# thilinarmtb/lsbench

Hardware: AMD Instinct MI355X
Metric: cg_solves_per_sec (higher is better)
Workload: dtype f64

## Files before the change

### include/lsbench_hip.h

```cpp
#ifndef LSBENCH_HIP_H
#define LSBENCH_HIP_H

#include "lsbench.h"
#include <stddef.h>

#ifdef __cplusplus
extern "C" {
#endif


struct lsbench {
  char *matrix;
  lsbench_solver_t solver;
  lsbench_ordering_t ordering;
  lsbench_precision_t precision;
  unsigned verbose, trials;
};

struct csr {
  unsigned nrows, base;
  unsigned *offs, *cols;
  double *vals;
};

// ... 49 lines not shown
  int overlap;
  int spmv_tune;
  int spmv_grid;
  int reorder;
  int krylov;
  int restart;
  int verbose;
  int ngpus;
  int verify;
  int cheb_degree;
  int block_size;
  int precision;
  int persistent;
  double comm_deadline_s;
  int fsai_power;
  int blas1_nt;
};
enum { LSB_PREC_FP64 = 0, LSB_PREC_MIXED = 1 };

struct lsb_hip_result {
  unsigned iters;
  int status;
  double relres;
  double seconds;
  double spmv_ms;
  unsigned spmv_samples;
  unsigned corrections;
  double true_relres;
  unsigned spmvs;
};

void lsb_hip_opts_default(struct lsb_hip_opts *o);
void lsb_hip_set_opts(const struct lsb_hip_opts *o);
void lsb_hip_get_opts(struct lsb_hip_opts *o);
void lsb_hip_last_result(struct lsb_hip_result *res);
int lsb_hip_device_count(void);


void lsb_csr_free(struct csr *A);
struct csr *lsb_csr_symmetrize_upper(const struct csr *A);
struct csr *lsb_csr_copy_base0(const struct csr *A);
struct csr *lsb_csr_row_slice(const struct csr *A, unsigned r0, unsigned r1);
int lsb_csr_partition_rows(const struct csr *A, unsigned nparts,
                           unsigned *bounds);
unsigned lsb_csr_row_blocks(const struct csr *A, unsigned cap,
                            unsigned **rowblk);
void lsb_csr_block_lanes(const struct csr *A, const unsigned *rowblk,
                         unsigned nblk, unsigned char *lanes);
struct csr *lsb_csr_pad_lines(const struct csr *S, unsigned slice, unsigned *nx, unsigned *nxp, int **map);
int lsb_csr_rcm(const struct csr *S, unsigned *perm);
struct csr *lsb_csr_permute_sym(const struct csr *S, const unsigned *perm);
unsigned lsb_csr_bandwidth(const struct csr *S);
struct lsb_panel_csr {
  unsigned npanels, width, npairs, nrows;
  unsigned *pair_begin;
  unsigned *pair_row;
  unsigned *offs;
  unsigned *cols;
  double *vals;
};
struct lsb_panel_csr *lsb_csr_panelize(const struct csr *A, unsigned width);
void lsb_panel_csr_free(struct lsb_panel_csr *P);
#define LSB_BIN_CHUNK 2048
struct lsb_binned {
  unsigned nbins, width, nrows, nchunks;
  unsigned chunk_cap;
  unsigned long long nnz;
  unsigned *bin_chunk;
  unsigned *chunk_begin;
  unsigned *rows;
  unsigned *cols;
  double *vals;
};
struct lsb_binned *lsb_csr_binize(const struct csr *A, unsigned width);
void lsb_binned_free(struct lsb_binned *B);
#define LSB_PB_COLS 8192
#define LSB_PB_ROWS 2048
struct lsb_pb {
  unsigned nrows, ncols_lo, nchunks, nbins, nitems, npieces;
  unsigned cols, rows;
  unsigned long long nnz;
  unsigned long long nent;
  double *vals;
  unsigned short *colw;
  unsigned *grp_first;
  unsigned long long *grp_mask;
  unsigned *delta;
  unsigned *item;
  unsigned *bin_ptr;
  unsigned short *roww;
};
struct lsb_pb *lsb_csr_pbize2(const struct csr *A, unsigned cols, unsigned rows);
struct lsb_pb *lsb_csr_pbize(const struct csr *A);
void lsb_pb_free(struct lsb_pb *P);
int lsb_pb_check(const struct lsb_pb *P, unsigned long long prod_len, unsigned long long roww_len, int deep,
                 char *why, size_t whylen);
struct lsb_fsai_pattern {
  unsigned n, cap;
  unsigned long long nnz;
  unsigned *offs, *cols;
};
#define LSB_FSAI_CAP 128
struct lsb_fsai_pattern *lsb_csr_fsai_pattern(const struct csr *S, int power, unsigned cap);
void lsb_fsai_pattern_free(struct lsb_fsai_pattern *P);
#define LSB_SELL_ROWS 128
struct lsb_sell {
  unsigned nrows, nslice;
  unsigned long long stored;
  unsigned *sptr;
  int *cols;
  double *vals;
  short *codes;
  int *sbase;
  unsigned ncode_slots;
};
unsigned long long lsb_csr_sell_stored(const struct csr *A);
struct lsb_sell *lsb_csr_sellize(const struct csr *A);
struct lsb_sell *lsb_csr_sellize16(const struct csr *A, unsigned row_begin);
void lsb_sell_free(struct lsb_sell *S);
struct lsb_sell_vc {
  unsigned long long nslots;
  unsigned nval_slots;
  int *slots;
  double *vconst;
  double *vals;
};
struct lsb_sell_vc *lsb_sell16_value_slots(const struct lsb_sell *S);
void lsb_sell_vc_free(struct lsb_sell_vc *V);
#define LSB_TMPL_SLOTS 8
struct lsb_sell_tmpl {
  int nslots;
  int shaped;
  int base[LSB_TMPL_SLOTS];
  int kidx[LSB_TMPL_SLOTS];
  int kind[LSB_TMPL_SLOTS];
  int pad_[2];
  double cst[LSB_TMPL_SLOTS];
};
struct lsb_sell_tmpls {
  unsigned nslice, ntmpl, nfar;
  unsigned long long covered, shaped;
  unsigned long long nmask;
  unsigned long long kept_read;
  unsigned char *tid;
  unsigned *vbase;
  unsigned long long *mask;
  struct lsb_sell_tmpl *t;
};
struct lsb_sell_tmpls *lsb_sell16_templates(const struct lsb_sell *S, const struct lsb_sell_vc *V);
void lsb_sell_tmpls_free(struct lsb_sell_tmpls *T);
int lsb_tmpl_check(const struct lsb_sell *S, const struct lsb_sell_vc *V, const struct lsb_sell_tmpls *T,
                   unsigned row_begin, unsigned nrows, unsigned xlen, int deep, char *why, size_t whylen);
#define LSB_TMPL_COL_MAX 16
#define LSB_TMPL_COL_LOCKSTEP 0x80000000u
struct lsb_tmpl_cols {
  unsigned nitem, kmax, period;
  unsigned s_lo, s_hi;
  unsigned xbeg[9];
  unsigned *item;
  unsigned long long in_cols;
  int centre0;
};
struct lsb_tmpl_cols *lsb_sell_tmpl_columns(const struct lsb_sell_tmpls *T, unsigned period, unsigned kmax);
struct lsb_tmpl_cols *lsb_sell_tmpl_columns_range(const struct lsb_sell_tmpls *T, unsigned period, unsigned kmax,
                                                  unsigned s_lo, unsigned s_hi);
void lsb_tmpl_cols_free(struct lsb_tmpl_cols *C);
int lsb_tmpl_cols_check(const struct lsb_sell_tmpls *T, const struct lsb_tmpl_cols *C, char *why, size_t whylen);
double lsb_csr_mean_scatter(const struct csr *A, unsigned row_begin);
void lsb_csr_col_hull(const struct csr *A, unsigned *lo, unsigned *hi);
struct lsb_xfer {
  int peer;
  size_t offset, count;
};
void lsb_plan_exchange(int me, int nall, const unsigned *hull,
                       struct lsb_xfer *recv, int *nrecv,
                       struct lsb_xfer *send, int *nsend);
struct csr *lsbench_matrix_synth(const char *spec, unsigned r0, unsigned r1,
                                 unsigned *n_global);


typedef struct lsb_hip_solver lsb_hip_solver;

lsb_hip_solver *lsb_hip_solver_create(const struct csr *A,
                                      const struct lsb_hip_opts *o);
lsb_hip_solver *lsb_hip_solver_create_dist(const struct csr *A_rows,
                                           unsigned row_begin,
                                           unsigned n_global,
                                           const struct lsb_hip_opts *o);
void lsb_hip_solver_destroy(lsb_hip_solver *s);

int lsb_hip_solver_solve(lsb_hip_solver *s, const double *b, double *x,
                         struct lsb_hip_result *res);
int lsb_hip_solver_solve_dev(lsb_hip_solver *s, const double *d_b, double *d_x,
                             struct lsb_hip_result *res);
int lsb_hip_solver_spmv_dev(lsb_hip_solver *s, const double *d_x, double *d_y);
int lsb_hip_solver_time_spmv(lsb_hip_solver *s, int warm, int reps,
                             double *ms_avg);
int lsb_hip_solver_jacobi_sweep_dev(lsb_hip_solver *s, double w,
                                    const double *d_b, double *d_x);

unsigned lsb_hip_solver_nrows_local(const lsb_hip_solver *s);
int lsb_hip_solver_padded(const lsb_hip_solver *s);
unsigned lsb_hip_solver_nrows_global(const lsb_hip_solver *s);
unsigned long long lsb_hip_solver_nnz_local(const lsb_hip_solver *s);
unsigned lsb_hip_solver_nblocks(const lsb_hip_solver *s);
int lsb_hip_solver_spmv_variant(const lsb_hip_solver *s);
unsigned lsb_hip_solver_spmv_flags(const lsb_hip_solver *s);
unsigned lsb_hip_solver_spmv_grid(const lsb_hip_solver *s);
unsigned lsb_hip_solver_spmv_period(const lsb_hip_solver *s);
unsigned long long lsb_hip_solver_spmv_col_slices(const lsb_hip_solver *s);
void lsb_hip_solver_sell_value_slots(const lsb_hip_solver *s, unsigned *kept, unsigned *total);
int lsb_hip_solver_overlaps(const lsb_hip_solver *s);
int lsb_hip_solver_comm(const lsb_hip_solver *s, double *p2p_us, double *rccl_us);
void lsb_hip_solver_comm_plan(const lsb_hip_solver *s, unsigned long long plan[8]);
int lsb_hip_solver_overlap(const lsb_hip_solver *s, double us[2]);
unsigned long long lsb_hip_solver_spmv_layout_bytes(const lsb_hip_solver *s);
unsigned long long lsb_hip_solver_iteration_bytes(const lsb_hip_solver *s);
int lsb_hip_solver_single_reduction(const lsb_hip_solver *s);
int lsb_hip_solver_fused_p(const lsb_hip_solver *s);
int lsb_hip_solver_blas1_nt(const lsb_hip_solver *s);
void *lsb_hip_stream(void);


#define LSB_HIP_UNIQUE_ID_BYTES 128
int lsb_hip_comm_get_unique_id(void *id128);
int lsb_hip_comm_init_rank(const void *id128, int nranks, int rank);
int lsb_hip_comm_destroy(void);
int lsb_hip_comm_rank(void);
int lsb_hip_comm_size(void);
int lsb_hip_comm_count(void);
int lsb_hip_comm_allreduce_sum_dev(double *d_buf, int count);
int lsb_hip_comm_barrier(void);


#define LSB_SPMV_FLAG_PREFETCH 1u
#define LSB_SPMV_FLAG_NT 2u
#define LSB_SPMV_FLAG_C16 4u
int lsb_hip_spmv_csr_f64(int variant, unsigned n, const int *d_offs,
                         const int *d_cols, const double *d_vals,
                         const int *d_rowblk, const unsigned char *d_blklanes,
                         unsigned nblk, unsigned mean_row_len, unsigned flags,
                         const double *d_x, double *d_y,
                         const double *d_xdot, double *d_dot, double *d_work,
                         void *stream);
unsigned lsb_hip_partials_capacity(void);
int lsb_hip_dot_f64(unsigned n, const double *d_a, const double *d_b,
                    double *d_out, double *d_work, void *stream);
int lsb_hip_nrm2_f64(unsigned n, const double *d_a, double *d_out,
                     double *d_work, void *stream);
int lsb_hip_axpy_f64(unsigned n, const double *d_alpha, const double *d_x,
                     double *d_y, void *stream);
int lsb_hip_xpay_f64(unsigned n, const double *d_beta, const double *d_x,
                     double *d_y, void *stream);
int lsb_hip_jacobi_setup_f64(unsigned n, unsigned row_begin, const int *d_offs,
                             const int *d_cols, const double *d_vals,
                             double *d_dinv, int *d_nzero, void *stream);
int lsb_hip_jacobi_apply_f64(unsigned n, const double *d_dinv,
                             const double *d_r, double *d_z, void *stream);

void *lsb_hip_malloc(size_t bytes);
void lsb_hip_free(void *d_ptr);
int lsb_hip_memcpy_h2d(void *d_dst, const void *src, size_t bytes);
int lsb_hip_memcpy_d2h(void *dst, const void *d_src, size_t bytes);
int lsb_hip_sync(void);

#ifdef __cplusplus
}
#endif

#endif
```

### lsbench_amd/_lib.py

```python
import ctypes as C
import os
import subprocess

_CSRC = os.path.join(os.path.dirname(os.path.abspath(__file__)), "csrc")
LIB_PATH = os.path.join(_CSRC, "liblsbench_hip.so")
CORE_PATH = os.path.join(_CSRC, "liblsbench_core.so")
CORE_SYMBOLS = ("lsbench_matrix_read", "lsbench_matrix_print", "lsbench_matrix_free", "lsbench_init",
                "lsbench_get_matrix_name", "lsbench_bench", "lsbench_finalize")

UNIQUE_ID_BYTES = 128

SOLVER_HIP = 6
OP_CHOLMOD_UPPER, OP_RAW = 0, 1
PRECOND_JACOBI, PRECOND_NONE, PRECOND_L1JACOBI, PRECOND_CHEBYSHEV, PRECOND_BLOCKJACOBI, PRECOND_FSAI = 0, 1, 2, 3, 4, 5
KRYLOV_PCG, KRYLOV_GMRES, KRYLOV_PCG1, KRYLOV_AUTO = 0, 1, 2, 3
SPMV_AUTO, SPMV_ADAPTIVE, SPMV_SUBWAVE, SPMV_SCALAR, SPMV_PANEL, SPMV_SELL, SPMV_BINNED, SPMV_TWOPHASE = 0, 1, 2, 3, 4, 5, 6, 7
SELL_ROWS = 128
BIN_CHUNK = 2048
PB_COLS, PB_ROWS = 8192, 2048
SPMV_FLAG_PREFETCH, SPMV_FLAG_NT, SPMV_FLAG_C16, SPMV_FLAG_TMPL, SPMV_FLAG_DEFER, SPMV_FLAG_COL = 1, 2, 4, 64, 128, 256
STATUS_RUNNING, STATUS_CONVERGED, STATUS_BREAKDOWN, STATUS_MAXIT = 0, 1, 2, 3
STATUS_COMM = 4
COMM_AUTO, COMM_RCCL, COMM_P2P = 0, 1, 2
PREC_FP64, PREC_MIXED = 0, 1


class LsbenchHipError(RuntimeError):
    pass


class CsrStruct(C.Structure):
    _fields_ = [("nrows", C.c_uint), ("base", C.c_uint),
                ("offs", C.POINTER(C.c_uint)), ("cols", C.POINTER(C.c_uint)),
                ("vals", C.POINTER(C.c_double))]


class LsbenchStruct(C.Structure):
    _fields_ = [("matrix", C.c_char_p), ("solver", C.c_int), ("ordering", C.c_int),
                ("precision", C.c_int), ("verbose", C.c_uint), ("trials", C.c_uint)]


class Opts(C.Structure):
    _fields_ = [("tol", C.c_double), ("maxit", C.c_uint), ("op_mode", C.c_int),
                ("precond", C.c_int), ("spmv_variant", C.c_int),
                ("check_every", C.c_int), ("use_graph", C.c_int),
                ("sample_spmv", C.c_int), ("nvirt", C.c_int), ("comm", C.c_int), ("overlap", C.c_int),
                ("spmv_tune", C.c_int), ("spmv_grid", C.c_int), ("reorder", C.c_int),
                ("krylov", C.c_int),
                ("restart", C.c_int), ("verbose", C.c_int),
                ("ngpus", C.c_int), ("verify", C.c_int), ("cheb_degree", C.c_int),
                ("block_size", C.c_int), ("precision", C.c_int), ("persistent", C.c_int),
                ("comm_deadline_s", C.c_double), ("fsai_power", C.c_int), ("blas1_nt", C.c_int)]


class Result(C.Structure):
    _fields_ = [("iters", C.c_uint), ("status", C.c_int), ("relres", C.c_double),
                ("seconds", C.c_double), ("spmv_ms", C.c_double),
                ("spmv_samples", C.c_uint), ("corrections", C.c_uint),
                ("true_relres", C.c_double), ("spmvs", C.c_uint)]


class PanelCsr(C.Structure):
    _fields_ = [("npanels", C.c_uint), ("width", C.c_uint), ("npairs", C.c_uint),
                ("nrows", C.c_uint), ("pair_begin", C.POINTER(C.c_uint)),
                ("pair_row", C.POINTER(C.c_uint)), ("offs", C.POINTER(C.c_uint)),
                ("cols", C.POINTER(C.c_uint)), ("vals", C.POINTER(C.c_double))]


class Sell(C.Structure):
    _fields_ = [("nrows", C.c_uint), ("nslice", C.c_uint), ("stored", C.c_ulonglong),
                ("sptr", C.POINTER(C.c_uint)), ("cols", C.POINTER(C.c_int)),
                ("vals", C.POINTER(C.c_double)), ("codes", C.POINTER(C.c_short)),
                ("sbase", C.POINTER(C.c_int)), ("ncode_slots", C.c_uint)]


class SellVc(C.Structure):
    _fields_ = [("nslots", C.c_ulonglong), ("nval_slots", C.c_uint), ("slots", C.POINTER(C.c_int)),
                ("vconst", C.POINTER(C.c_double)), ("vals", C.POINTER(C.c_double))]


class FsaiPattern(C.Structure):
    _fields_ = [("n", C.c_uint), ("cap", C.c_uint), ("nnz", C.c_ulonglong), ("offs", C.POINTER(C.c_uint)),
                ("cols", C.POINTER(C.c_uint))]


class SellTmpl(C.Structure):
    _fields_ = [("nslots", C.c_int), ("shaped", C.c_int), ("base", C.c_int * 8), ("kidx", C.c_int * 8),
                ("kind", C.c_int * 8), ("pad_", C.c_int * 2), ("cst", C.c_double * 8)]


class SellTmpls(C.Structure):
    _fields_ = [("nslice", C.c_uint), ("ntmpl", C.c_uint), ("nfar", C.c_uint), ("covered", C.c_ulonglong),
                ("shaped", C.c_ulonglong), ("nmask", C.c_ulonglong), ("kept_read", C.c_ulonglong),
                ("tid", C.POINTER(C.c_ubyte)), ("vbase", C.POINTER(C.c_uint)),
                ("mask", C.POINTER(C.c_ulonglong)), ("t", C.POINTER(SellTmpl))]


class TmplCols(C.Structure):
    _fields_ = [("nitem", C.c_uint), ("kmax", C.c_uint), ("period", C.c_uint), ("s_lo", C.c_uint), ("s_hi", C.c_uint),
                ("xbeg", C.c_uint * 9),
                ("item", C.POINTER(C.c_uint)), ("in_cols", C.c_ulonglong), ("centre0", C.c_int)]


class Binned(C.Structure):
    _fields_ = [("nbins", C.c_uint), ("width", C.c_uint), ("nrows", C.c_uint), ("nchunks", C.c_uint),
                ("chunk_cap", C.c_uint), ("nnz", C.c_ulonglong), ("bin_chunk", C.POINTER(C.c_uint)),
                ("chunk_begin", C.POINTER(C.c_uint)), ("rows", C.POINTER(C.c_uint)),
                ("cols", C.POINTER(C.c_uint)), ("vals", C.POINTER(C.c_double))]


class Pb(C.Structure):
    _fields_ = [("nrows", C.c_uint), ("ncols_lo", C.c_uint), ("nchunks", C.c_uint), ("nbins", C.c_uint),
                ("nitems", C.c_uint), ("npieces", C.c_uint), ("cols", C.c_uint), ("rows", C.c_uint),
                ("nnz", C.c_ulonglong), ("nent", C.c_ulonglong),
                ("vals", C.POINTER(C.c_double)), ("colw", C.POINTER(C.c_ushort)),
                ("grp_first", C.POINTER(C.c_uint)), ("grp_mask", C.POINTER(C.c_ulonglong)),
                ("delta", C.POINTER(C.c_uint)), ("item", C.POINTER(C.c_uint)),
                ("bin_ptr", C.POINTER(C.c_uint)), ("roww", C.POINTER(C.c_ushort))]


class Xfer(C.Structure):
    _fields_ = [("peer", C.c_int), ("offset", C.c_size_t), ("count", C.c_size_t)]


_vp, _u, _i, _d = C.c_void_p, C.c_uint, C.c_int, C.c_double
_csrp = C.POINTER(CsrStruct)

SIGNATURES = {
    "lsbench_matrix_read": (_csrp, [C.c_char_p]),
    "lsbench_matrix_print": (None, [_csrp]),
    "lsbench_matrix_free": (None, [_csrp]),
    "lsbench_init": (C.POINTER(LsbenchStruct), [_i, C.POINTER(C.c_char_p)]),
    "lsbench_get_matrix_name": (C.c_char_p, [C.POINTER(LsbenchStruct)]),
    "lsbench_bench": (None, [_csrp, C.POINTER(LsbenchStruct)]),
    "lsbench_finalize": (None, [C.POINTER(LsbenchStruct)]),
    "hip_cdna4_init": (_i, []),
    "hip_cdna4_finalize": (_i, []),
    "hip_cdna4_bench": (_i, [C.POINTER(C.c_double), _csrp, C.POINTER(C.c_double),
                             C.POINTER(LsbenchStruct)]),
    "lsb_hip_opts_default": (None, [C.POINTER(Opts)]),
    "lsb_hip_set_opts": (None, [C.POINTER(Opts)]),
    "lsb_hip_get_opts": (None, [C.POINTER(Opts)]),
    "lsb_hip_last_result": (None, [C.POINTER(Result)]),
    "lsb_hip_device_count": (_i, []),
    "lsb_csr_free": (None, [_csrp]),
    "lsb_csr_symmetrize_upper": (_csrp, [_csrp]),
    "lsb_csr_copy_base0": (_csrp, [_csrp]),
    "lsb_csr_row_slice": (_csrp, [_csrp, _u, _u]),
    "lsb_csr_partition_rows": (_i, [_csrp, _u, C.POINTER(_u)]),
    "lsb_csr_row_blocks": (_u, [_csrp, _u, C.POINTER(C.POINTER(_u))]),
    "lsb_csr_block_lanes": (None, [_csrp, C.POINTER(_u), _u, C.POINTER(C.c_ubyte)]),
    "lsb_csr_rcm": (_i, [_csrp, C.POINTER(_u)]),
    "lsb_csr_permute_sym": (_csrp, [_csrp, C.POINTER(_u)]),
    "lsb_csr_bandwidth": (_u, [_csrp]),
    "lsb_csr_panelize": (C.POINTER(PanelCsr), [_csrp, _u]),
    "lsb_panel_csr_free": (None, [C.POINTER(PanelCsr)]),
    "lsb_csr_pbize": (C.POINTER(Pb), [_csrp]),
    "lsb_csr_pbize2": (C.POINTER(Pb), [_csrp, _u, _u]),
    "lsb_pb_free": (None, [C.POINTER(Pb)]),
    "lsb_pb_check": (_i, [C.POINTER(Pb), C.c_ulonglong, C.c_ulonglong, _i, C.c_char_p, C.c_size_t]),
    "lsb_csr_binize": (C.POINTER(Binned), [_csrp, _u]),
    "lsb_binned_free": (None, [C.POINTER(Binned)]),
    "lsb_csr_sell_stored": (C.c_ulonglong, [_csrp]),
    "lsb_csr_sellize": (C.POINTER(Sell), [_csrp]),
    "lsb_csr_sellize16": (C.POINTER(Sell), [_csrp, _u]),
    "lsb_sell_free": (None, [C.POINTER(Sell)]),
    "lsb_sell16_value_slots": (C.POINTER(SellVc), [C.POINTER(Sell)]),
    "lsb_sell_vc_free": (None, [C.POINTER(SellVc)]),
    "lsb_csr_fsai_pattern": (C.POINTER(FsaiPattern), [_csrp, _i, _u]),
    "lsb_fsai_pattern_free": (None, [C.POINTER(FsaiPattern)]),
    "lsb_sell16_templates": (C.POINTER(SellTmpls), [C.POINTER(Sell), C.POINTER(SellVc)]),
    "lsb_sell_tmpls_free": (None, [C.POINTER(SellTmpls)]),
    "lsb_tmpl_check": (_i, [C.POINTER(Sell), C.POINTER(SellVc), C.POINTER(SellTmpls), _u, _u, _u, _i,
                            C.c_char_p, C.c_size_t]),
    "lsb_sell_tmpl_columns": (C.POINTER(TmplCols), [C.POINTER(SellTmpls), _u, _u]),
    "lsb_sell_tmpl_columns_range": (C.POINTER(TmplCols), [C.POINTER(SellTmpls), _u, _u, _u, _u]),
    "lsb_tmpl_cols_free": (None, [C.POINTER(TmplCols)]),
    "lsb_tmpl_cols_check": (_i, [C.POINTER(SellTmpls), C.POINTER(TmplCols), C.c_char_p, C.c_size_t]),
    "lsb_csr_mean_scatter": (_d, [_csrp, _u]),
    "lsb_csr_col_hull": (None, [_csrp, C.POINTER(_u), C.POINTER(_u)]),
    "lsb_plan_exchange": (None, [_i, _i, C.POINTER(_u), C.POINTER(Xfer), C.POINTER(_i),
                                 C.POINTER(Xfer), C.POINTER(_i)]),
    "lsbench_matrix_synth": (_csrp, [C.c_char_p, _u, _u, C.POINTER(_u)]),
    "lsb_hip_solver_create": (_vp, [_csrp, C.POINTER(Opts)]),
    "lsb_hip_solver_create_dist": (_vp, [_csrp, _u, _u, C.POINTER(Opts)]),
    "lsb_hip_solver_destroy": (None, [_vp]),
    "lsb_hip_solver_solve": (_i, [_vp, _vp, _vp, C.POINTER(Result)]),
    "lsb_hip_solver_solve_dev": (_i, [_vp, _vp, _vp, C.POINTER(Result)]),
    "lsb_hip_solver_spmv_dev": (_i, [_vp, _vp, _vp]),
    "lsb_hip_solver_time_spmv": (_i, [_vp, _i, _i, C.POINTER(_d)]),
    "lsb_hip_solver_jacobi_sweep_dev": (_i, [_vp, _d, _vp, _vp]),
    "lsb_hip_solver_nrows_local": (_u, [_vp]),
    "lsb_hip_solver_padded": (_i, [_vp]),
    "lsb_csr_pad_lines": (_csrp, [_csrp, _u, C.POINTER(_u), C.POINTER(_u), C.POINTER(C.POINTER(C.c_int))]),
    "lsb_hip_solver_nrows_global": (_u, [_vp]),
    "lsb_hip_solver_nnz_local": (C.c_ulonglong, [_vp]),
    "lsb_hip_solver_nblocks": (_u, [_vp]),
    "lsb_hip_solver_spmv_variant": (_i, [_vp]),
    "lsb_hip_solver_spmv_flags": (_u, [_vp]),
    "lsb_hip_solver_spmv_grid": (_u, [_vp]),
    "lsb_hip_solver_spmv_period": (_u, [_vp]),
    "lsb_hip_solver_spmv_col_slices": (C.c_ulonglong, [_vp]),
    "lsb_hip_solver_sell_value_slots": (None, [_vp, C.POINTER(C.c_uint), C.POINTER(C.c_uint)]),
    "lsb_hip_solver_overlaps": (_i, [_vp]),
    "lsb_hip_solver_overlap": (_i, [_vp, C.POINTER(C.c_double)]),
    "lsb_hip_solver_comm_plan": (None, [_vp, C.POINTER(C.c_ulonglong)]),
    "lsb_hip_solver_spmv_layout_bytes": (C.c_ulonglong, [_vp]),
    "lsb_hip_solver_fused_p": (_i, [_vp]),
    "lsb_hip_solver_iteration_bytes": (C.c_ulonglong, [_vp]),
    "lsb_hip_solver_single_reduction": (_i, [_vp]),
    "lsb_hip_solver_blas1_nt": (_i, [_vp]),
    "lsb_hip_solver_comm": (_i, [_vp, C.POINTER(C.c_double), C.POINTER(C.c_double)]),
    "lsb_hip_stream": (_vp, []),
    "lsb_hip_comm_get_unique_id": (_i, [_vp]),
    "lsb_hip_comm_init_rank": (_i, [_vp, _i, _i]),
    "lsb_hip_comm_destroy": (_i, []),
    "lsb_hip_comm_rank": (_i, []),
    "lsb_hip_comm_size": (_i, []),
    "lsb_hip_comm_count": (_i, []),
    "hip_cdna4_set_option": (_i, [C.c_char_p, C.c_char_p]),
    "hip_cdna4_matrix_synth": (_csrp, [C.c_char_p]),
    "lsb_hip_comm_allreduce_sum_dev": (_i, [_vp, _i]),
    "lsb_hip_comm_barrier": (_i, []),
    "lsb_hip_spmv_csr_f64": (_i, [_i, _u, _vp, _vp, _vp, _vp, _vp, _u, _u, _u, _vp, _vp,
                                  _vp, _vp, _vp, _vp]),
    "lsb_hip_partials_capacity": (_u, []),
    "lsb_hip_dot_f64": (_i, [_u, _vp, _vp, _vp, _vp, _vp]),
    "lsb_hip_nrm2_f64": (_i, [_u, _vp, _vp, _vp, _vp]),
    "lsb_hip_axpy_f64": (_i, [_u, _vp, _vp, _vp, _vp]),
    "lsb_hip_xpay_f64": (_i, [_u, _vp, _vp, _vp, _vp]),
    "lsb_hip_jacobi_setup_f64": (_i, [_u, _u, _vp, _vp, _vp, _vp, _vp, _vp]),
    "lsb_hip_jacobi_apply_f64": (_i, [_u, _vp, _vp, _vp, _vp]),
    "lsb_hip_malloc": (_vp, [C.c_size_t]),
    "lsb_hip_free": (None, [_vp]),
    "lsb_hip_memcpy_h2d": (_i, [_vp, _vp, C.c_size_t]),
    "lsb_hip_memcpy_d2h": (_i, [_vp, _vp, C.c_size_t]),
    "lsb_hip_sync": (_i, []),
}

_LIB = None


def build(force=False):
    if force:
        subprocess.run(["make", "-s", "-C", _CSRC, "clean"], check=True)
    subprocess.run(["make", "-s", "-C", _CSRC, "all"], check=True)


def libc_free(ptr):
    libc = C.CDLL(None)
    libc.free.argtypes, libc.free.restype = [C.c_void_p], None
    libc.free(C.cast(ptr, C.c_void_p))


# ... 34 lines not shown
```

### lsbench_amd/csrc/hip_kernels.hip

```cpp
#include <hip/hip_runtime.h>
#include <stdint.h>
#include <string.h>

#include "hip_ar.h"
#include "lsb_impl.h"

#include "hip_wg.h"
static_assert(WG == AR_WG, "the folded all-reduce phases assume this workgroup size");

__device__ __forceinline__ void spmv_publish(double *__restrict__ partials, double dot,
                                             double *sred, const lsb_ar_tail &tail) {
  if (!partials)
    return;
  double d[1] = {dot};
  wg_sum<1>(d, sred);
  if (tail.counter)
    ar_tail(partials, d[0], tail);
  else if (threadIdx.x == 0)
    partials[blockIdx.x] = d[0];
}

enum { SP_PREFETCH = 1, SP_NT = 2 };

template <int FLAGS, class T>
// ... 1169 lines not shown
      if (!have_xd && !(dot_is_x && bc == 0)) {
        if (row + 1 < n)
          xd = *(const sell_d2v *)(xdot + row);
        else if (row < n)
          xd.x = xdot[row];
        have_xd = true;
      }
      unsigned long long mk[2][2] = {{0ull, 0ull}, {0ull, 0ull}};
#pragma unroll
      for (int side = 0; side < 2; side++)
        if (side_k[side] >= 0 && side_kd[side] == 2) {
          const unsigned long long *mp = mask + 2 * ((size_t)mb + (unsigned)side_k[side]);
          mk[side][0] = mp[0], mk[side][1] = mp[1];
        }
      TMPL_UNPARK();
      if (stopped)
        return;
      double up = lane_above(c.y), dn = lane_below(c.x);
      if (lane == 0)
        up = edge;
      if (lane == 63)
        dn = edge;
      if (!have_xd)
        xd.x = c.x, xd.y = c.y, have_xd = true;
#pragma unroll
      for (int k = 0; k < NF; k++) {
        const double v = T->cst[k];
        a0 = fma(v, lo[k].x, a0), a1 = fma(v, lo[k].y, a1);
      }
      {
        double vm0 = T->cst[NF], vm1 = vm0, vp0 = T->cst[NF + 2], vp1 = vp0;
        if (side_k[0] >= 0 || side_k[1] >= 0)
          tmpl_side_values(T, NF, vb, lane, side_k, side_kd, mk, vals, f32, vm0, vm1, vp0, vp1);
        const double vc = T->cst[NF + 1];
        a0 = fma(vm0, vm0 != 0.0 ? up : 0.0, a0), a1 = fma(vm1, vm1 != 0.0 ? c.x : 0.0, a1);
        a0 = fma(vc, c.x, a0), a1 = fma(vc, c.y, a1);
        a0 = fma(vp0, vp0 != 0.0 ? c.y : 0.0, a0), a1 = fma(vp1, vp1 != 0.0 ? dn : 0.0, a1);
      }
#pragma unroll
      for (int k = 0; k < NF; k++) {
        const double v = T->cst[NF + 3 + k];
        a0 = fma(v, hi[k].x, a0), a1 = fma(v, hi[k].y, a1);
      }
    } else {
      TMPL_UNPARK();
      if (!have_xd) {
        if (row + 1 < n)
          xd = *(const sell_d2v *)(xdot + row);
        else if (row < n)
          xd.x = xdot[row];
        have_xd = true;
      }
      if (t != 255u) {
        const int cnt = T->nslots;
        if (stopped)
          return;
        for (int u0 = 0; u0 < LSB_TMPL_SLOTS; u0 += 4) {
          sell_d2u v[4];
#pragma unroll
          for (int u = 0; u < 4; u++)
            if (u0 + u < cnt)
              v[u] = *(const sell_d2u *)(x + (grow + T->base[u0 + u]));
#pragma unroll
          for (int u = 0; u < 4; u++)
            if (u0 + u < cnt) {
              const double k = T->cst[u0 + u];
              a0 = fma(k, v[u].x, a0), a1 = fma(k, v[u].y, a1);
            }
        }
      } else {
        const unsigned q0 = sptr[s] / LSB_SELL_ROWS, len = (sptr[s + 1] - sptr[s]) / LSB_SELL_ROWS;
        if (stopped)
          return;
        for (unsigned j = 0; j < len; j++) {
          const i4v r = ((const i4v *)sbase)[q0 + j];
          if (r.z < 0) {
            const double k = vconst[q0 + j];
            const sell_d2u v = *(const sell_d2u *)(x + (grow + r.x));
            a0 = fma(k, v.x, a0), a1 = fma(k, v.y, a1);
          } else {
            double v0, v1;
            if (f32) {
              const vt2<float>::type v = *((const vt2<float>::type *)((const float *)vals + (size_t)r.z * LSB_SELL_ROWS) + lane);
              v0 = (double)v.x, v1 = (double)v.y;
            } else {
              const sell_d2v v = *((const sell_d2v *)((const double *)vals + (size_t)r.z * LSB_SELL_ROWS) + lane);
              v0 = v.x, v1 = v.y;
            }
            const bool p0 = v0 != 0.0, p1 = v1 != 0.0;
            const double t0 = x[p0 ? grow + r.x : 0], t1 = x[p1 ? grow + 1 + r.x : 0];
            a0 = fma(v0, p0 ? t0 : 0.0, a0), a1 = fma(v1, p1 ? t1 : 0.0, a1);
          }
        }
      }
    }
    if (CHEB) {
      if (row + 1 < n) {
        const sell_d2v rr = *(const sell_d2v *)(epi.r + row), dd = *(const sell_d2v *)(epi.d + row);
        const double i0 = epi.dinv ? epi.dinv[row] : epi.dc, i1 = epi.dinv ? epi.dinv[row + 1] : epi.dc;
        const double v0 = fma(epi.a, dd.x, epi.b * (i0 * (rr.x - a0)));
        const double v1 = fma(epi.a, dd.y, epi.b * (i1 * (rr.y - a1)));
        const sell_d2v dn2 = {v0, v1}, zn = {x[grow] + v0, x[grow + 1] + v1};
        *(sell_d2v *)(epi.d + row) = dn2;
        *(sell_d2v *)(epi.zout + row) = zn;
      } else if (row < n) {
        const double v0 = fma(epi.a, epi.d[row], epi.b * ((epi.dinv ? epi.dinv[row] : epi.dc) * (epi.r[row] - a0)));
        epi.d[row] = v0;
        epi.zout[row] = x[grow] + v0;
      }
    } else if (DEFER && s * LSB_SELL_ROWS + LSB_SELL_ROWS <= n) {
      const sell_d2v o = {a0, a1};
      if (DEFER_DEPTH == 1 || pslot == 0)
        ypark[tid] = o, parked[0] = s * LSB_SELL_ROWS;
      else
        ypark[(DEFER_DEPTH - 1) * WG + tid] = o, parked[DEFER_DEPTH - 1] = s * LSB_SELL_ROWS;
      if (xdot) {
        dot = fma(a0, xd.x, dot);
        dot = fma(a1, xd.y, dot);
      }
    } else if (row + 1 < n) {
      const sell_d2v o = {a0, a1};
      *(sell_d2v *)(y + row) = o;
      if (xdot) {
        dot = fma(a0, xd.x, dot);
        dot = fma(a1, xd.y, dot);
      }
    } else if (row < n) {
      y[row] = a0;
      if (xdot)
        dot = fma(a0, xd.x, dot);
    }
  }
#pragma unroll
  for (int k = 0; k < DEFER_DEPTH; k++)
    TMPL_UNPARK_SLOT(k);
#undef TMPL_UNPARK
#undef TMPL_UNPARK_SLOT
  if (stopped)
    return;
  spmv_publish(partials, dot, sred, tail);
}

template <int NF> struct col_ops {
  sell_d2u lo[NF > 1 ? NF - 1 : 1], hi[NF > 1 ? NF - 1 : 1];
  double edge;
  sell_d2v xd;
};
template <int NF> struct col_tmpl {
  int bc, bl[NF > 1 ? NF - 1 : 1], bh[NF > 1 ? NF - 1 : 1];
  double k0, kl[NF > 1 ? NF - 1 : 1], kc, kh[NF > 1 ? NF - 1 : 1], kL;
};
template <int NF, int DOT>
__device__ __forceinline__ void col_issue(col_ops<NF> &o, sell_d2u &cnext, const col_tmpl<NF> &T, const double *__restrict__ x,
                                          const double *__restrict__ xdot, long long gu, unsigned lrow, unsigned P,
                                          unsigned xlen, unsigned lane, bool with_next) {
  if (with_next)
    cnext = *(const sell_d2u *)(x + (gu + T.bc + (long long)P) + 2 * lane);
#pragma unroll
  for (int k = 0; k < NF - 1; k++) {
    o.lo[k] = *(const sell_d2u *)(x + (gu + T.bl[k]) + 2 * lane);
    o.hi[k] = *(const sell_d2u *)(x + (gu + T.bh[k]) + 2 * lane);
  }
  long long el = gu + T.bc - 1, er = gu + T.bc + (long long)LSB_SELL_ROWS;
  el = el < 0 ? 0 : el, er = er >= (long long)xlen ? (long long)xlen - 1 : er;
  o.edge = x[lane < 32u ? el : er];
  if (DOT == 2)
    o.xd = *(const sell_d2v *)(xdot + lrow + 2 * lane);
}
template <int NF, int DOT>
__device__ __forceinline__ void col_compute(const col_ops<NF> &o, const sell_d2u &cm, const sell_d2u &c, const sell_d2u &cp,
                                            const col_tmpl<NF> &T, double vm0, double vm1, double vp0, double vp1,
                                            unsigned lane, double &a0, double &a1, double &dot) {
  double up = lane_above(c.y), dn = lane_below(c.x);
  if (lane == 0)
    up = o.edge;
  if (lane == 63)
    dn = o.edge;
  a0 = fma(T.k0, cm.x, 0.0), a1 = fma(T.k0, cm.y, 0.0);
#pragma unroll
  for (int k = 0; k < NF - 1; k++)
    a0 = fma(T.kl[k], o.lo[k].x, a0), a1 = fma(T.kl[k], o.lo[k].y, a1);
  a0 = fma(vm0, vm0 != 0.0 ? up : 0.0, a0), a1 = fma(vm1, vm1 != 0.0 ? c.x : 0.0, a1);
  a0 = fma(T.kc, c.x, a0), a1 = fma(T.kc, c.y, a1);
  a0 = fma(vp0, vp0 != 0.0 ? c.y : 0.0, a0), a1 = fma(vp1, vp1 != 0.0 ? dn : 0.0, a1);
#pragma unroll
  for (int k = 0; k < NF - 1; k++)
    a0 = fma(T.kh[k], o.hi[k].x, a0), a1 = fma(T.kh[k], o.hi[k].y, a1);
  a0 = fma(T.kL, cp.x, a0), a1 = fma(T.kL, cp.y, a1);
  if (DOT == 1)
    dot = fma(a0, c.x, dot), dot = fma(a1, c.y, dot);
  else if (DOT == 2)
    dot = fma(a0, o.xd.x, dot), dot = fma(a1, o.xd.y, dot);
}

#define LSB_COL_HEAD 16
template <int NF, int DOT>
__global__ __launch_bounds__(WG, DOT == 2 ? 5 : 6) void k_spmv_tmpl_col(
    const unsigned *__restrict__ plan, unsigned period, unsigned n, unsigned row_begin, unsigned xlen,
    const unsigned *__restrict__ sptr, const unsigned long long *__restrict__ mask,
    const lsb_sell_tmpl *__restrict__ td, const int *__restrict__ sbase, const void *__restrict__ vals, int f32,
    const double *__restrict__ vconst, const double *__restrict__ x, double *__restrict__ y,
    const double *__restrict__ xdot, double *__restrict__ partials, const lsb_pcg_state *__restrict__ st,
    const lsb_ar_tail tail) {
  static_assert(NF >= 1 && NF <= 2, "one or two far slots per side");
  __shared__ double sred[4];
  const unsigned tid = threadIdx.x, lane = tid & 63u, wave = tid >> 6;
  const unsigned gx = gridDim.x / NXCD, xcd = blockIdx.x % NXCD, slot = blockIdx.x / NXCD;
  const unsigned i0 = plan[xcd], i1 = plan[xcd + 1];
  const u4v *__restrict__ items = (const u4v *)(plan + LSB_COL_HEAD);
  const int stopped = st ? st->status : 0;
  const unsigned P = period * LSB_SELL_ROWS;
  double dot = 0.0;
  for (unsigned g = slot; i0 + 4 * g < i1; g += gx) {
    const unsigned it = __builtin_amdgcn_readfirstlane(i0 + 4 * g + wave);
    if (it >= i1)
      continue;
    const u4v rec = items[it];
    const unsigned s = __builtin_amdgcn_readfirstlane(rec.x), Kw = __builtin_amdgcn_readfirstlane(rec.y);
    const unsigned K = Kw & ~LSB_TMPL_COL_LOCKSTEP;
    const bool lockstep = (Kw & LSB_TMPL_COL_LOCKSTEP) != 0;
    if (K >= 2) {
      const unsigned t = __builtin_amdgcn_readfirstlane(rec.z), mb = __builtin_amdgcn_readfirstlane(rec.w);
      const lsb_sell_tmpl *T = td + t;
      col_tmpl<NF> C;
      C.bc = T->base[NF + 1];
      C.k0 = T->cst[0], C.kc = T->cst[NF + 1], C.kL = T->cst[2 * NF + 2];
#pragma unroll
      for (int k = 0; k < NF - 1; k++) {
        C.bl[k] = T->base[1 + k], C.bh[k] = T->base[NF + 3 + k];
        C.kl[k] = T->cst[1 + k], C.kh[k] = T->cst[NF + 3 + k];
      }
      const int side_k[2] = {T->kidx[NF], T->kidx[NF + 2]}, side_kd[2] = {T->kind[NF], T->kind[NF + 2]};
      long long gu = (long long)s * LSB_SELL_ROWS + row_begin;
      unsigned lrow = s * LSB_SELL_ROWS;
      col_ops<NF> cur, nxt;
      sell_d2u cm = *(const sell_d2u *)(x + (gu + C.bc - (long long)P) + 2 * lane);
      sell_d2u c0 = *(const sell_d2u *)(x + (gu + C.bc) + 2 * lane);
      sell_d2u cp, cn;
      col_issue<NF, DOT>(cur, cp, C, x, xdot, gu, lrow, P, xlen, lane, true);
      unsigned long long mk[2][2] = {{0ull, 0ull}, {0ull, 0ull}};
#pragma unroll
      for (int side = 0; side < 2; side++)
        if (side_k[side] >= 0 && side_kd[side] == 2) {
          const unsigned long long *mp = mask + 2 * ((size_t)mb + (unsigned)side_k[side]);
          mk[side][0] = mp[0], mk[side][1] = mp[1];
        }
      double vm0 = T->cst[NF], vm1 = vm0, vp0 = T->cst[NF + 2], vp1 = vp0;
      if (side_k[0] >= 0 || side_k[1] >= 0)
        tmpl_side_values(T, NF, 0u, lane, side_k, side_kd, mk, vals, f32, vm0, vm1, vp0, vp1);
      if (stopped)
        return;
      col_issue<NF, DOT>(nxt, cn, C, x, xdot, gu + (long long)P, lrow + P, P, xlen, lane, true);
      double a0, a1;
      col_compute<NF, DOT>(cur, cm, c0, cp, C, vm0, vm1, vp0, vp1, lane, a0, a1, dot);
      cm = c0, c0 = cp, cp = cn, cur = nxt;
      for (unsigned k = 1; k + 1 < K; k++) {
        gu += (long long)P, lrow += P;
        if (lockstep)
          __builtin_amdgcn_s_barrier();
        col_issue<NF, DOT>(nxt, cn, C, x, xdot, gu + (long long)P, lrow + P, P, xlen, lane, true);
        {
          const sell_d2v o = {a0, a1};
          *(sell_d2v *)(y + (lrow - P) + 2 * lane) = o;
        }
        col_compute<NF, DOT>(cur, cm, c0, cp, C, vm0, vm1, vp0, vp1, lane, a0, a1, dot);
        cm = c0, c0 = cp, cp = cn, cur = nxt;
      }
      gu += (long long)P, lrow += P;
      {
        const sell_d2v o = {a0, a1};
        *(sell_d2v *)(y + (lrow - P) + 2 * lane) = o;
      }
      col_compute<NF, DOT>(cur, cm, c0, cp, C, vm0, vm1, vp0, vp1, lane, a0, a1, dot);
      {
        const sell_d2v o = {a0, a1};
        *(sell_d2v *)(y + lrow + 2 * lane) = o;
      }
    } else {
      const unsigned row = s * LSB_SELL_ROWS + 2 * lane;
      const int grow = (int)(row + row_begin);
      const unsigned q0 = sptr[s] / LSB_SELL_ROWS, len = (sptr[s + 1] - sptr[s]) / LSB_SELL_ROWS;
      sell_d2v xd = {0.0, 0.0};
      if (DOT) {
        if (row + 1 < n)
          xd = *(const sell_d2v *)(xdot + row);
        else if (row < n)
          xd.x = xdot[row];
      }
      if (stopped)
        return;
      double a0 = 0.0, a1 = 0.0;
      for (unsigned j = 0; j < len; j++) {
        const i4v r = ((const i4v *)sbase)[q0 + j];
        if (r.z < 0) {
          const double k = vconst[q0 + j];
          const sell_d2u v = *(const sell_d2u *)(x + (grow + r.x));
          a0 = fma(k, v.x, a0), a1 = fma(k, v.y, a1);
        } else {
          double v0, v1;
          if (f32) {
            const vt2<float>::type v = *((const vt2<float>::type *)((const float *)vals + (size_t)r.z * LSB_SELL_ROWS) + lane);
            v0 = (double)v.x, v1 = (double)v.y;
          } else {
            const sell_d2v v = *((const sell_d2v *)((const double *)vals + (size_t)r.z * LSB_SELL_ROWS) + lane);
            v0 = v.x, v1 = v.y;
          }
          const bool p0 = v0 != 0.0, p1 = v1 != 0.0;
          const double t0 = x[p0 ? grow + r.x : 0], t1 = x[p1 ? grow + 1 + r.x : 0];
          a0 = fma(v0, p0 ? t0 : 0.0, a0), a1 = fma(v1, p1 ? t1 : 0.0, a1);
        }
      }
      if (row + 1 < n) {
        const sell_d2v o = {a0, a1};
        *(sell_d2v *)(y + row) = o;
        if (DOT)
          dot = fma(a0, xd.x, dot), dot = fma(a1, xd.y, dot);
      } else if (row < n) {
        y[row] = a0;
        if (DOT)
          dot = fma(a0, xd.x, dot);
      }
    }
  }
  if (stopped)
    return;
  spmv_publish(partials, dot, sred, tail);
}

template <int NF> struct colp_c {
  sell_d2u rn, pn;
  sell_d2v xn, sn;
  double re, pe;
};
template <int NF> struct colp_m {
  sell_d2u rlo[NF > 1 ? NF - 1 : 1], plo[NF > 1 ? NF - 1 : 1], rhi[NF > 1 ? NF - 1 : 1], phi[NF > 1 ? NF - 1 : 1];
};
struct colp_out {
  sell_d2v q, x, p;
};
template <int NF, bool WITH_X, int NT>
__device__ __forceinline__ void colp_issue_c(colp_c<NF> &o, const col_tmpl<NF> &T, const double *__restrict__ r,
                                             const double *__restrict__ pold, const double *__restrict__ x,
                                             const double *pstale, long long gu, unsigned P, unsigned xlen,
                                             unsigned lane) {
  const long long ga = gu + T.bc + (long long)P;
  o.rn = *(const sell_d2u *)(r + ga + 2 * lane);
  o.pn = *(const sell_d2u *)(pold + ga + 2 * lane);
  if (WITH_X) {
    if (NT & 1) {
      o.xn = __builtin_nontemporal_load((const sell_d2v *)(x + (gu + (long long)P) + 2 * lane));
      o.sn = __builtin_nontemporal_load((const sell_d2v *)(pstale + (gu + (long long)P) + 2 * lane));
    } else {
      o.xn = *(const sell_d2v *)(x + (gu + (long long)P) + 2 * lane);
      o.sn = *(const sell_d2v *)(pstale + (gu + (long long)P) + 2 * lane);
    }
  }
  long long el = gu + T.bc - 1, er = gu + T.bc + (long long)LSB_SELL_ROWS;
  el = el < 0 ? 0 : el, er = er >= (long long)xlen ? (long long)xlen - 1 : er;
  const long long e = lane < 32u ? el : er;
  o.re = r[e], o.pe = pold[e];
}
template <int NF>
__device__ __forceinline__ void colp_issue_m(colp_m<NF> &o, const col_tmpl<NF> &T, const double *__restrict__ r,
                                             const double *__restrict__ pold, long long gu, unsigned lane) {
#pragma unroll
  for (int k = 0; k < NF - 1; k++) {
    o.rlo[k] = *(const sell_d2u *)(r + (gu + T.bl[k]) + 2 * lane);
    o.plo[k] = *(const sell_d2u *)(pold + (gu + T.bl[k]) + 2 * lane);
    o.rhi[k] = *(const sell_d2u *)(r + (gu + T.bh[k]) + 2 * lane);
    o.phi[k] = *(const sell_d2u *)(pold + (gu + T.bh[k]) + 2 * lane);
  }
}
template <int NF, bool OWNED, bool XUPD>
__device__ __forceinline__ void colp_compute(const colp_c<NF> &o, const colp_m<NF> &m, const sell_d2u &pm,
                                             const sell_d2u &p0, sell_d2u &pp, const col_tmpl<NF> &T, double vm0,
                                             double vm1, double vp0, double vp1, double beta, double alpha, double alpha2,
                                             double dc, unsigned lane, colp_out &out, double &dot) {
  pp.x = pnew_of(dc, o.rn.x, beta, o.pn.x), pp.y = pnew_of(dc, o.rn.y, beta, o.pn.y);
  if (OWNED) {
    if (XUPD) {
      out.x.x = (o.xn.x + alpha2 * o.sn.x) + alpha * o.pn.x, out.x.y = (o.xn.y + alpha2 * o.sn.y) + alpha * o.pn.y;
    }
    out.p.x = pp.x, out.p.y = pp.y;
  }
  const double edge = pnew_of(dc, o.re, beta, o.pe);
  double up = lane_above(p0.y), dn = lane_below(p0.x);
  if (lane == 0)
    up = edge;
  if (lane == 63)
    dn = edge;
  double a0 = fma(T.k0, pm.x, 0.0), a1 = fma(T.k0, pm.y, 0.0);
#pragma unroll
  for (int k = 0; k < NF - 1; k++) {
    const double l0 = pnew_of(dc, m.rlo[k].x, beta, m.plo[k].x), l1 = pnew_of(dc, m.rlo[k].y, beta, m.plo[k].y);
    a0 = fma(T.kl[k], l0, a0), a1 = fma(T.kl[k], l1, a1);
  }
  a0 = fma(vm0, vm0 != 0.0 ? up : 0.0, a0), a1 = fma(vm1, vm1 != 0.0 ? p0.x : 0.0, a1);
  a0 = fma(T.kc, p0.x, a0), a1 = fma(T.kc, p0.y, a1);
  a0 = fma(vp0, vp0 != 0.0 ? p0.y : 0.0, a0), a1 = fma(vp1, vp1 != 0.0 ? dn : 0.0, a1);
#pragma unroll
  for (int k = 0; k < NF - 1; k++) {
    const double h0 = pnew_of(dc, m.rhi[k].x, beta, m.phi[k].x), h1 = pnew_of(dc, m.rhi[k].y, beta, m.phi[k].y);
    a0 = fma(T.kh[k], h0, a0), a1 = fma(T.kh[k], h1, a1);
  }
  a0 = fma(T.kL, pp.x, a0), a1 = fma(T.kL, pp.y, a1);
  out.q.x = a0, out.q.y = a1;
  dot = fma(a0, p0.x, dot), dot = fma(a1, p0.y, dot);
}
__device__ __forceinline__ void colp_single(unsigned s, unsigned n, unsigned lane, const unsigned *__restrict__ sptr,
                                            const int *__restrict__ sbase, const double *__restrict__ vals,
                                            const double *__restrict__ vconst, const double *__restrict__ r,
                                            const double *__restrict__ pold, double *pnew,
                                            double *__restrict__ x, double *__restrict__ q, double beta, double alpha,
                                            double alpha2, bool xupd, double dc, double &dot) {
  const unsigned row = s * LSB_SELL_ROWS + 2 * lane;
  const unsigned q0 = sptr[s] / LSB_SELL_ROWS, len = (sptr[s + 1] - sptr[s]) / LSB_SELL_ROWS;
  const bool l0 = row < n, l1 = row + 1 < n;
  const double r0 = l0 ? r[row] : 0.0, r1 = l1 ? r[row + 1] : 0.0;
  const double o0 = l0 ? pold[row] : 0.0, o1 = l1 ? pold[row + 1] : 0.0;
  const double x0 = xupd && l0 ? x[row] : 0.0, x1 = xupd && l1 ? x[row + 1] : 0.0;
  const double s0 = xupd && l0 ? pnew[row] : 0.0, s1 = xupd && l1 ? pnew[row + 1] : 0.0;
  double a0 = 0.0, a1 = 0.0;
  for (unsigned j = 0; j < len; j++) {
    const i4v rec = ((const i4v *)sbase)[q0 + j];
    if (rec.z < 0) {
      const double k = vconst[q0 + j];
      const sell_d2u rv = *(const sell_d2u *)(r + ((int)row + rec.x)), pv = *(const sell_d2u *)(pold + ((int)row + rec.x));
      a0 = fma(k, pnew_of(dc, rv.x, beta, pv.x), a0), a1 = fma(k, pnew_of(dc, rv.y, beta, pv.y), a1);
    } else {
      const sell_d2v v = *((const sell_d2v *)(vals + (size_t)rec.z * LSB_SELL_ROWS) + lane);
      const bool p0 = v.x != 0.0, p1 = v.y != 0.0;
      const int c0 = p0 ? (int)row + rec.x : 0, c1 = p1 ? (int)row + 1 + rec.x : 0;
      const double t0 = pnew_of(dc, r[c0], beta, pold[c0]), t1 = pnew_of(dc, r[c1], beta, pold[c1]);
      a0 = fma(v.x, p0 ? t0 : 0.0, a0), a1 = fma(v.y, p1 ? t1 : 0.0, a1);
    }
  }
  const double n0 = pnew_of(dc, r0, beta, o0), n1 = pnew_of(dc, r1, beta, o1);
  if (l0) {
    pnew[row] = n0;
    if (xupd)
      x[row] = (x0 + alpha2 * s0) + alpha * o0;
    if (q)
      q[row] = a0;
    dot = fma(a0, n0, dot);
  }
  if (l1) {
    pnew[row + 1] = n1;
    if (xupd)
      x[row + 1] = (x1 + alpha2 * s1) + alpha * o1;
    if (q)
      q[row + 1] = a1;
    dot = fma(a1, n1, dot);
  }
}

#define COLP_ST(PTR, V, BIT)                                                                   \
  do {                                                                                         \
    if (NT & (BIT))                                                                            \
      __builtin_nontemporal_store((V), (sell_d2v *)(PTR));                                     \
    else                                                                                       \
      *(sell_d2v *)(PTR) = (V);                                                                \
  } while (0)
#define COLP_STORE(OUT, LROW, WITH_Q, WITH_XP)                                                 \
  do {                                                                                         \
    if (WITH_Q)                                                                                \
      COLP_ST(q + (LROW) + 2 * lane, (OUT).q, 2);                                              \
    if (WITH_XP) {                                                                             \
      if (XUPD)                                                                                \
        COLP_ST(x + ((LROW) + P) + 2 * lane, (OUT).x, 1);                                      \
      COLP_ST(pnew + ((LROW) + P) + 2 * lane, (OUT).p, 2);                                     \
    }                                                                                          \
  } while (0)

template <int NF, int NT, bool XUPD>
__global__ __launch_bounds__(WG, NF == 2 ? 3 : 4) void k_pcg_col_px(
    const unsigned *__restrict__ plan, unsigned period, unsigned n, const unsigned *__restrict__ sptr,
    const unsigned long long *__restrict__ mask, const lsb_sell_tmpl *__restrict__ td, const int *__restrict__ sbase,
    const double *__restrict__ vals, const double *__restrict__ vconst, const double *__restrict__ r,
    const double *__restrict__ pold, double *pnew, double *__restrict__ x, double dc,
    double *__restrict__ partials, lsb_pcg_state *__restrict__ st, int parity,
    const double *__restrict__ parts2, unsigned nparts2) {
  static_assert(NF >= 1 && NF <= 2, "one or two far slots per side");
  __shared__ double sred[8];
  double *const q = nullptr;
  const unsigned tid = threadIdx.x, lane = tid & 63u, wave = tid >> 6;
  const unsigned gx = gridDim.x / NXCD, xcd = blockIdx.x % NXCD, slot = blockIdx.x / NXCD;
  const int stopped = st->status;
  const double rz_old = st->rz[parity], thresh2 = st->thresh2, alpha = st->alpha[0], alpha2 = st->alpha[1];
  const unsigned i0 = plan[xcd], i1 = plan[xcd + 1];
  double v[2];
  wg_sum_partials<2>(parts2, nparts2, v, sred);
  if (stopped)
    return;
  const double rz_new = v[0], rr = v[1];
  const bool conv = rr <= thresh2;
  if (blockIdx.x == 0 && threadIdx.x == 0) {
    const int it = st->iters + 1;
    st->iters = it;
    st->rr = rr;
    st->rz[parity ^ 1] = rz_new;
    if (conv)
      st->status = LSB_STATUS_CONVERGED;
    else {
      if (XUPD)
        st->xpend = 0;
      if (it >= st->maxit)
        st->pad = 1;
    }
  }
  if (conv)
    return;
  const double beta = rz_new / rz_old;
  const u4v *__restrict__ items = (const u4v *)(plan + LSB_COL_HEAD);
  const unsigned P = period * LSB_SELL_ROWS;
  double dot = 0.0;
  for (unsigned g = slot; i0 + 4 * g < i1; g += gx) {
    const unsigned it = __builtin_amdgcn_readfirstlane(i0 + 4 * g + wave);
    if (it >= i1)
      continue;
    const u4v rec = items[it];
    const unsigned s = __builtin_amdgcn_readfirstlane(rec.x);
    const unsigned K = __builtin_amdgcn_readfirstlane(rec.y) & ~LSB_TMPL_COL_LOCKSTEP;
    if (K >= 3) {
      const unsigned t = __builtin_amdgcn_readfirstlane(rec.z), mb = __builtin_amdgcn_readfirstlane(rec.w);
      const lsb_sell_tmpl *T = td + t;
      col_tmpl<NF> C;
      C.bc = T->base[NF + 1];
      C.k0 = T->cst[0], C.kc = T->cst[NF + 1], C.kL = T->cst[2 * NF + 2];
#pragma unroll
      for (int k = 0; k < NF - 1; k++) {
        C.bl[k] = T->base[1 + k], C.bh[k] = T->base[NF + 3 + k];
        C.kl[k] = T->cst[1 + k], C.kh[k] = T->cst[NF + 3 + k];
      }
      const int side_k[2] = {T->kidx[NF], T->kidx[NF + 2]}, side_kd[2] = {T->kind[NF], T->kind[NF + 2]};
      long long gu = (long long)s * LSB_SELL_ROWS;
      unsigned lrow = s * LSB_SELL_ROWS;
      const long long gc = gu + C.bc;
      const sell_d2u rb = *(const sell_d2u *)(r + (gc - (long long)P) + 2 * lane);
      const sell_d2u pb = *(const sell_d2u *)(pold + (gc - (long long)P) + 2 * lane);
      const sell_d2u r0 = *(const sell_d2u *)(r + gc + 2 * lane), o0 = *(const sell_d2u *)(pold + gc + 2 * lane);
      sell_d2v x0 = {0.0, 0.0}, s0 = {0.0, 0.0};
      if (XUPD)
        x0 = *(const sell_d2v *)(x + lrow + 2 * lane), s0 = *(const sell_d2v *)(pnew + lrow + 2 * lane);
      colp_c<NF> c0, c1;
      colp_m<NF> m0, m1, m2;
      colp_issue_c<NF, XUPD, NT>(c0, C, r, pold, x, pnew, gu, P, n, lane);
      colp_issue_m<NF>(m0, C, r, pold, gu, lane);
      colp_issue_m<NF>(m1, C, r, pold, gu + (long long)P, lane);
      unsigned long long mk[2][2] = {{0ull, 0ull}, {0ull, 0ull}};
#pragma unroll
      for (int side = 0; side < 2; side++)
        if (side_k[side] >= 0 && side_kd[side] == 2) {
          const unsigned long long *mp = mask + 2 * ((size_t)mb + (unsigned)side_k[side]);
          mk[side][0] = mp[0], mk[side][1] = mp[1];
        }
      double vm0 = T->cst[NF], vm1 = vm0, vp0 = T->cst[NF + 2], vp1 = vp0;
      if (side_k[0] >= 0 || side_k[1] >= 0)
        tmpl_side_values(T, NF, 0u, lane, side_k, side_kd, mk, vals, 0, vm0, vm1, vp0, vp1);
      sell_d2u pm, p0, pp;
      pm.x = pnew_of(dc, rb.x, beta, pb.x), pm.y = pnew_of(dc, rb.y, beta, pb.y);
      p0.x = pnew_of(dc, r0.x, beta, o0.x), p0.y = pnew_of(dc, r0.y, beta, o0.y);
      colp_out res;
      res.x.x = (x0.x + alpha2 * s0.x) + alpha * o0.x, res.x.y = (x0.y + alpha2 * s0.y) + alpha * o0.y;
      res.p.x = p0.x, res.p.y = p0.y;
      res.q = res.p;
      COLP_STORE(res, lrow - P, false, true);
      for (unsigned k = 0; k + 2 < K; k++) {
        colp_issue_c<NF, XUPD, NT>(c1, C, r, pold, x, pnew, gu + (long long)P, P, n, lane);
        colp_issue_m<NF>(m2, C, r, pold, gu + 2 * (long long)P, lane);
        colp_compute<NF, true, XUPD>(c0, m0, pm, p0, pp, C, vm0, vm1, vp0, vp1, beta, alpha, alpha2, dc, lane, res, dot);
        COLP_STORE(res, lrow, false, true);
        pm = p0, p0 = pp, c0 = c1, m0 = m1, m1 = m2;
        gu += (long long)P, lrow += P;
      }
      colp_issue_c<NF, false, NT>(c1, C, r, pold, x, pnew, gu + (long long)P, P, n, lane);
      colp_compute<NF, true, XUPD>(c0, m0, pm, p0, pp, C, vm0, vm1, vp0, vp1, beta, alpha, alpha2, dc, lane, res, dot);
      COLP_STORE(res, lrow, false, true);
      pm = p0, p0 = pp, c0 = c1, m0 = m1;
      gu += (long long)P, lrow += P;
      colp_compute<NF, false, XUPD>(c0, m0, pm, p0, pp, C, vm0, vm1, vp0, vp1, beta, alpha, alpha2, dc, lane, res, dot);
      COLP_STORE(res, lrow, false, false);
    } else {
      for (unsigned k = 0; k < K; k++)
        colp_single(s + k * period, n, lane, sptr, sbase, vals, vconst, r, pold, pnew, x, nullptr, beta, alpha, alpha2,
                    XUPD, dc, dot);
    }
  }
  if (partials) {
    double d[1] = {dot};
    wg_sum<1>(d, sred);
    if (threadIdx.x == 0)
      partials[blockIdx.x] = d[0];
  }
}
#undef COLP_STORE
#undef COLP_ST

template <int NF>
__global__ __launch_bounds__(WG, 5) void k_pcg_col_r(
    const unsigned *__restrict__ plan, unsigned period, unsigned n, const unsigned *__restrict__ sptr,
    const unsigned long long *__restrict__ mask, const lsb_sell_tmpl *__restrict__ td, const int *__restrict__ sbase,
    const double *__restrict__ vals, const double *__restrict__ vconst, const double *__restrict__ p,
    double *__restrict__ r, double dc, lsb_pcg_state *__restrict__ st, int parity, int pbuf, int xtwo,
    const double *__restrict__ pq_parts, unsigned npq, double *__restrict__ partials2) {
  static_assert(NF >= 1 && NF <= 2, "one or two far slots per side");
  __shared__ double sred[8];
  const unsigned tid = threadIdx.x, lane = tid & 63u, wave = tid >> 6;
  const unsigned gx = gridDim.x / NXCD, xcd = blockIdx.x % NXCD, slot = blockIdx.x / NXCD;
  const int stopped = st->status, pad = st->pad;
  const double rz = st->rz[parity];
  const unsigned i0 = plan[xcd], i1 = plan[xcd + 1];
  double pqv[1];
  wg_sum_partials<1>(pq_parts, npq, pqv, sred);
  if (stopped)
    return;
  if (pad) {
    if (blockIdx.x == 0 && threadIdx.x == 0)
      st->status = LSB_STATUS_MAXIT;
    return;
  }
  const double pq = pqv[0];
  if (!(pq != 0.0) || !isfinite(pq)) {
    if (blockIdx.x == 0 && threadIdx.x == 0)
      st->status = LSB_STATUS_BREAKDOWN;
    return;
  }
  const double alpha = rz / pq;
  if (blockIdx.x == 0 && threadIdx.x == 0) {
    st->pq = pq, st->alpha[1] = st->alpha[0], st->alpha[0] = alpha, st->xpend = (xtwo ? 3 : 1) + pbuf;
  }
  const u4v *__restrict__ items = (const u4v *)(plan + LSB_COL_HEAD);
  const unsigned P = period * LSB_SELL_ROWS;
  double acc[2] = {0.0, 0.0}, nodot = 0.0;
#define COLR_FINISH(A0, A1, RV, LROW)                                                          \
  do {                                                                                         \
    sell_d2v rn_;                                                                              \
    rn_.x = (RV).x - alpha * (A0), rn_.y = (RV).y - alpha * (A1);                              \
    *(sell_d2v *)(r + (LROW) + 2 * lane) = rn_;                                                \
    acc[0] += rn_.x * (dc * rn_.x);                                                            \
    acc[0] += rn_.y * (dc * rn_.y);                                                            \
    acc[1] += rn_.x * rn_.x;                                                                   \
    acc[1] += rn_.y * rn_.y;                                                                   \
  } while (0)
  for (unsigned g = slot; i0 + 4 * g < i1; g += gx) {
    const unsigned it = __builtin_amdgcn_readfirstlane(i0 + 4 * g + wave);
    if (it >= i1)
      continue;
    const u4v rec = items[it];
    const unsigned s = __builtin_amdgcn_readfirstlane(rec.x);
    const unsigned K = __builtin_amdgcn_readfirstlane(rec.y) & ~LSB_TMPL_COL_LOCKSTEP;
    if (K >= 3) {
      const unsigned t = __builtin_amdgcn_readfirstlane(rec.z), mb = __builtin_amdgcn_readfirstlane(rec.w);
      const lsb_sell_tmpl *T = td + t;
      col_tmpl<NF> C;
      C.bc = T->base[NF + 1];
      C.k0 = T->cst[0], C.kc = T->cst[NF + 1], C.kL = T->cst[2 * NF + 2];
#pragma unroll
      for (int k = 0; k < NF - 1; k++) {
        C.bl[k] = T->base[1 + k], C.bh[k] = T->base[NF + 3 + k];
        C.kl[k] = T->cst[1 + k], C.kh[k] = T->cst[NF + 3 + k];
      }
      const int side_k[2] = {T->kidx[NF], T->kidx[NF + 2]}, side_kd[2] = {T->kind[NF], T->kind[NF + 2]};
      long long gu = (long long)s * LSB_SELL_ROWS;
      unsigned lrow = s * LSB_SELL_ROWS;
      col_ops<NF> cur, nxt;
      sell_d2u cm = *(const sell_d2u *)(p + (gu + C.bc - (long long)P) + 2 * lane);
      sell_d2u c0 = *(const sell_d2u *)(p + (gu + C.bc) + 2 * lane);
      sell_d2u cp, cn;
      col_issue<NF, 2>(cur, cp, C, p, r, gu, lrow, P, n, lane, true);
      unsigned long long mk[2][2] = {{0ull, 0ull}, {0ull, 0ull}};
#pragma unroll
      for (int side = 0; side < 2; side++)
        if (side_k[side] >= 0 && side_kd[side] == 2) {
          const unsigned long long *mp = mask + 2 * ((size_t)mb + (unsigned)side_k[side]);
          mk[side][0] = mp[0], mk[side][1] = mp[1];
        }
      double vm0 = T->cst[NF], vm1 = vm0, vp0 = T->cst[NF + 2], vp1 = vp0;
      if (side_k[0] >= 0 || side_k[1] >= 0)
        tmpl_side_values(T, NF, 0u, lane, side_k, side_kd, mk, vals, 0, vm0, vm1, vp0, vp1);
      for (unsigned k = 0; k + 1 < K; k++) {
        col_issue<NF, 2>(nxt, cn, C, p, r, gu + (long long)P, lrow + P, P, n, lane, true);
        double a0, a1;
        col_compute<NF, 0>(cur, cm, c0, cp, C, vm0, vm1, vp0, vp1, lane, a0, a1, nodot);
        COLR_FINISH(a0, a1, cur.xd, lrow);
        cm = c0, c0 = cp, cp = cn, cur = nxt;
        gu += (long long)P, lrow += P;
      }
      double a0, a1;
      col_compute<NF, 0>(cur, cm, c0, cp, C, vm0, vm1, vp0, vp1, lane, a0, a1, nodot);
      COLR_FINISH(a0, a1, cur.xd, lrow);
    } else {
      for (unsigned k = 0; k < K; k++) {
        const unsigned sl = s + k * period, row = sl * LSB_SELL_ROWS + 2 * lane;
        const unsigned q0 = sptr[sl] / LSB_SELL_ROWS, len = (sptr[sl + 1] - sptr[sl]) / LSB_SELL_ROWS;
        const bool l0 = row < n, l1 = row + 1 < n;
        const double r0 = l0 ? r[row] : 0.0, r1 = l1 ? r[row + 1] : 0.0;
        double a0 = 0.0, a1 = 0.0;
        for (unsigned j = 0; j < len; j++) {
          const i4v rec2 = ((const i4v *)sbase)[q0 + j];
          if (rec2.z < 0) {
            const double kk = vconst[q0 + j];
            const sell_d2u pv = *(const sell_d2u *)(p + ((int)row + rec2.x));
            a0 = fma(kk, pv.x, a0), a1 = fma(kk, pv.y, a1);
          } else {
            const sell_d2v v = *((const sell_d2v *)(vals + (size_t)rec2.z * LSB_SELL_ROWS) + lane);
            const bool p0 = v.x != 0.0, p1 = v.y != 0.0;
            const double t0 = p[p0 ? (int)row + rec2.x : 0], t1 = p[p1 ? (int)row + 1 + rec2.x : 0];
            a0 = fma(v.x, p0 ? t0 : 0.0, a0), a1 = fma(v.y, p1 ? t1 : 0.0, a1);
          }
        }
        if (l0) {
          const double rn0 = r0 - alpha * a0;
          r[row] = rn0;
          acc[0] += rn0 * (dc * rn0), acc[1] += rn0 * rn0;
        }
        if (l1) {
          const double rn1 = r1 - alpha * a1;
          r[row + 1] = rn1;
          acc[0] += rn1 * (dc * rn1), acc[1] += rn1 * rn1;
        }
      }
    }
  }
#undef COLR_FINISH
  wg_sum<2>(acc, sred);
  if (threadIdx.x == 0) {
    partials2[2 * blockIdx.x + 0] = acc[0];
    partials2[2 * blockIdx.x + 1] = acc[1];
  }
}

__global__ __launch_bounds__(WG) void k_pcg_xfix(unsigned n, const double *__restrict__ p0, const double *__restrict__ p1,
                                                 double *__restrict__ x, const lsb_pcg_state *__restrict__ st) {
  const int pend = st->xpend;
  if (!pend)
    return;
  const double alpha = st->alpha[0], alpha2 = st->alpha[1];
  if (pend <= 2) {
    const double *__restrict__ p = pend == 1 ? p0 : p1;
    for (size_t i = (size_t)blockIdx.x * WG + threadIdx.x; i < n; i += (size_t)gridDim.x * WG)
      x[i] += alpha * p[i];
  } else {
    const double *__restrict__ p = pend == 3 ? p0 : p1, *__restrict__ pp = pend == 3 ? p1 : p0;
    for (size_t i = (size_t)blockIdx.x * WG + threadIdx.x; i < n; i += (size_t)gridDim.x * WG)
      x[i] = (x[i] + alpha2 * pp[i]) + alpha * p[i];
  }
}

__device__ __forceinline__ unsigned bin_pad(unsigned i) { return i + (i >> 3); }

template <int FLAGS, int BIN_U>
__global__ __launch_bounds__(WG) void k_spmv_binned(
    const unsigned *__restrict__ chunk_begin, unsigned nchunk, const unsigned *__restrict__ rows,
    const unsigned *__restrict__ cols, const double *__restrict__ vals,
    const double *__restrict__ x, double *__restrict__ y, const lsb_pcg_state *__restrict__ st) {
  constexpr unsigned CHUNK = BIN_U * WG;
  __shared__ double sprod[CHUNK + CHUNK / 8 + 8];
  __shared__ unsigned skey[CHUNK + CHUNK / 8 + 8];
  __shared__ double swv[4];
  __shared__ int swf[4];
  __shared__ double sred[4];
  const unsigned tid = threadIdx.x, lane = tid & 63u, wave = tid >> 6;
  const unsigned per = gridDim.x / NXCD;
  const unsigned w = (blockIdx.x % NXCD) * per + blockIdx.x / NXCD;
  if (w >= nchunk)
    return;
  const unsigned e0 = chunk_begin[w], cnt = chunk_begin[w + 1] - e0;
  unsigned r[BIN_U], c[BIN_U];
  double v[BIN_U];
  if (cnt <= CHUNK) {
#pragma unroll
    for (int u = 0; u < BIN_U; u++) {
      const unsigned t = tid + u * WG;
      if (t < cnt) {
        r[u] = stream_load<FLAGS>(rows + e0 + t);
        c[u] = stream_load<FLAGS>(cols + e0 + t);
        v[u] = stream_load<FLAGS>(vals + e0 + t);
      }
    }
  }
  if (st && st->status)
    return;
  if (cnt > CHUNK) {
    double s[1] = {0.0};
    for (unsigned j = e0 + tid; j < e0 + cnt; j += WG)
      s[0] += vals[j] * x[cols[j]];
    wg_sum<1>(s, sred);
    if (tid == 0)
      y[rows[e0]] += s[0];
    return;
  }
#pragma unroll
  for (int u = 0; u < BIN_U; u++) {
    const unsigned t = tid + u * WG;
    if (t < cnt) {
      double xv;
      if (FLAGS & 8)
        xv = __hip_atomic_load(x + c[u], __ATOMIC_RELAXED, __HIP_MEMORY_SCOPE_AGENT);
      else if (FLAGS & 16)
        xv = __builtin_nontemporal_load(x + c[u]);
      else
        xv = x[c[u]];
      sprod[bin_pad(t)] = v[u] * xv;
      skey[bin_pad(t)] = r[u];
    }
  }
  __syncthreads();
  const unsigned i0 = tid * BIN_U;
  const int nloc = i0 < cnt ? (int)min(cnt - i0, (unsigned)BIN_U) : 0;
  double first_sum = 0.0, acc = 0.0;
  unsigned first_key = 0, prevk = 0xFFFFFFFFu, nextk = 0xFFFFFFFEu;
  bool cont = false, has_boundary = false, closes = true;
  unsigned ok_[BIN_U];
  double ov[BIN_U];
  unsigned omask = 0;
  if (nloc > 0) {
    if (i0 > 0)
      prevk = skey[bin_pad(i0 - 1)];
    if (i0 + BIN_U < cnt)
      nextk = skey[bin_pad(i0 + BIN_U)];
    unsigned k[BIN_U + 1];
    double p[BIN_U];
#pragma unroll
    for (int j = 0; j < BIN_U; j++) {
      k[j] = j < nloc ? skey[bin_pad(i0 + j)] : 0u;
      p[j] = j < nloc ? sprod[bin_pad(i0 + j)] : 0.0;
    }
    cont = k[0] == prevk;
    first_key = k[0];
#pragma unroll
    for (int j = 0; j < BIN_U; j++)
      if (j < nloc) {
        acc += p[j];
        const bool last = j == nloc - 1;
        const bool ends = last ? (k[j] != nextk) : (k[j + 1] != k[j]);
        if (last)
          closes = ends;
        if (ends) {
          if (cont && !has_boundary) {
            first_sum = acc;
          } else {
            omask |= 1u << j;
// ... 353 lines not shown
  const int dot = !partials || !xdot ? 0 : (xdot == x + row_begin && centre0) ? 1 : 2;
#define LSB_COL(NF, D)                                                                                \
  k_spmv_tmpl_col<NF, D><<<g, WG, 0, s>>>(plan, period, n, row_begin, xlen, sptr, mask, td, sbase, vals, f32, vconst, x, y, \
                                          xdot, partials, st, tail)
#define LSB_COLD(NF)                                                                                  \
  do {                                                                                                \
    if (dot == 0)                                                                                     \
      LSB_COL(NF, 0);                                                                                 \
    else if (dot == 1)                                                                                \
      LSB_COL(NF, 1);                                                                                 \
    else                                                                                              \
      LSB_COL(NF, 2);                                                                                 \
  } while (0)
  switch (nfar) {
  case 1: LSB_COLD(1); break;
  case 2: LSB_COLD(2); break;
  default: errx(EXIT_FAILURE, "lsb_k_spmv_tmpl_col: %u far slots per side", nfar);
  }
#undef LSB_COLD
#undef LSB_COL
}

void lsb_k_reduce_final(const double *partials, unsigned nparts, unsigned width,
                        double *out, int take_sqrt,
                        const struct lsb_pcg_state *st, void *stream) {
  k_reduce_final<<<1, WG, 0, (hipStream_t)stream>>>(partials, nparts, width, out,
                                                    take_sqrt, st);
}

void lsb_k_reduce_final2(const double *pa, unsigned na, unsigned wa, double *outa,
                         const double *pb, unsigned nb, unsigned wb, double *outb,
                         const struct lsb_pcg_state *st, void *stream) {
  k_reduce_final2<<<1, WG, 0, (hipStream_t)stream>>>(pa, na, wa, outa, pb, nb, wb, outb, st);
}

void lsb_k_dot(unsigned n, const double *a, const double *b, double *partials,
               unsigned *npartials, void *stream) {
  unsigned g = div_up(n ? n : 1, WG * 4);
  if (g > LSB_STREAM_GRID_CAP)
    g = LSB_STREAM_GRID_CAP;
  *npartials = g;
  k_dot<<<g, WG, 0, (hipStream_t)stream>>>(n, a, b, partials);
}

static unsigned ew_grid(unsigned n) {
  unsigned g = div_up(n ? n : 1, WG * 4);
  return g > LSB_STREAM_GRID_CAP ? LSB_STREAM_GRID_CAP : g;
}

void lsb_k_axpy(unsigned n, const double *alpha, const double *x, double *y,
                void *stream) {
  k_axpy<<<ew_grid(n), WG, 0, (hipStream_t)stream>>>(n, alpha, x, y);
}

void lsb_k_xpay(unsigned n, const double *beta, const double *x, double *y,
                void *stream) {
  k_xpay<<<ew_grid(n), WG, 0, (hipStream_t)stream>>>(n, beta, x, y);
}

void lsb_k_jacobi_setup(unsigned n, unsigned row_begin, const int *offs,
                        const int *cols, const double *vals, double *dinv,
                        int *nzero, void *stream) {
  k_jacobi_setup<<<ew_grid(n), WG, 0, (hipStream_t)stream>>>(n, row_begin, offs, cols,
                                                             vals, dinv, nzero);
}

void lsb_k_l1_setup(unsigned n, const int *offs, const double *vals, double *dinv, int *nzero,
                    void *stream) {
  k_l1_setup<<<ew_grid(n), WG, 0, (hipStream_t)stream>>>(n, offs, vals, dinv, nzero);
}

void lsb_k_jacobi_apply(unsigned n, const double *dinv, const double *r,
                        double *z, void *stream) {
  k_jacobi_apply<<<ew_grid(n), WG, 0, (hipStream_t)stream>>>(n, dinv, r, z);
}

void lsb_k_jacobi_sweep(unsigned n, double w, const double *dinv,
                        const double *b, const double *ax, double *x,
                        void *stream) {
  k_jacobi_sweep<<<ew_grid(n), WG, 0, (hipStream_t)stream>>>(n, w, dinv, b, ax, x);
}

void lsb_k_vreduce(double *base, unsigned stride, unsigned nshard, unsigned off,
                   unsigned cnt, void *stream) {
  k_vreduce<<<1, 64, 0, (hipStream_t)stream>>>(base, stride, nshard, off, cnt);
}

void lsb_k_perm_gather(unsigned n, const int *perm, const double *src, double *dst,
                       void *stream) {
  k_perm_gather<<<ew_grid(n), WG, 0, (hipStream_t)stream>>>(n, perm, src, dst);
}

void lsb_k_perm_scatter(unsigned n, const int *perm, const double *src, double *dst,
                        void *stream) {
  k_perm_scatter<<<ew_grid(n), WG, 0, (hipStream_t)stream>>>(n, perm, src, dst);
}

void lsb_k_fill_index(unsigned n, unsigned first, double *v, void *stream) {
  k_fill_index<<<ew_grid(n), WG, 0, (hipStream_t)stream>>>(n, first, v);
}

void lsb_k_pcg_init(unsigned n, const double *b, const double *dinv, double dc, double *x,
                    double *r, double *p, double *partials2,
                    unsigned *npartials, void *stream) {
  const unsigned g = lsb_k_blas1_grid(n);
  *npartials = g;
  if (aligned16(b) && aligned16(dinv) && aligned16(x) && aligned16(r) && aligned16(p))
    k_pcg_init<true><<<g, WG, 0, (hipStream_t)stream>>>(n, b, dinv, dc, x, r, p, partials2);
  else
    k_pcg_init<false><<<g, WG, 0, (hipStream_t)stream>>>(n, b, dinv, dc, x, r, p, partials2);
}

void lsb_k_pcg_init_state(struct lsb_pcg_state *st, const double *partials2,
                          unsigned nparts, double tol, int maxit,
                          void *stream) {
  k_pcg_init_state<<<1, WG, 0, (hipStream_t)stream>>>(st, partials2, nparts, tol, maxit);
}

void lsb_k_pcg_update_xr(unsigned n, const double *p, const double *q,
                         const double *dinv, double dc, double *x, double *r,
                         struct lsb_pcg_state *st, int parity,
                         const double *pq_parts, unsigned npq,
                         double *partials2, unsigned *npartials, void *stream) {
  const unsigned g = lsb_k_blas1_grid(n);
  *npartials = g;
  if (aligned16(p) && aligned16(q) && aligned16(dinv) && aligned16(x) && aligned16(r)) {
#define LSB_XR(A, B, C)                                                                           \
  k_pcg_update_xr<true, A, B, C><<<g, WG, 0, (hipStream_t)stream>>>(n, p, q, dinv, dc, x, r, st, parity, pq_parts, \
                                                                  npq, partials2)
    switch (g_blas1_nt & 7) {
    case 0: LSB_XR(false, false, false); break;
    case 1: LSB_XR(true, false, false); break;
    case 2: LSB_XR(false, true, false); break;
    case 3: LSB_XR(true, true, false); break;
    case 4: LSB_XR(false, false, true); break;
    case 5: LSB_XR(true, false, true); break;
    case 6: LSB_XR(false, true, true); break;
    default: LSB_XR(true, true, true); break;
    }
#undef LSB_XR
  } else {
    k_pcg_update_xr<false, false, false, false><<<g, WG, 0, (hipStream_t)stream>>>(
        n, p, q, dinv, dc, x, r, st, parity, pq_parts, npq, partials2);
  }
}

void lsb_k_pcg_col_px(unsigned grid_cap, unsigned period, const unsigned *plan, unsigned nitem, unsigned n,
                      const unsigned *sptr, const unsigned long long *mask, const struct lsb_sell_tmpl *td,
                      unsigned nfar, const int *sbase, const double *vals, const double *vconst, const double *r,
                      const double *pold, double *pnew, double *x, int xupd, double dc, double *partials,
                      unsigned *npartials, struct lsb_pcg_state *st, int parity, const double *parts2,
                      unsigned nparts2, void *stream) {
  hipStream_t s = (hipStream_t)stream;
  const unsigned res = nfar == 2 ? 768u : 1280u;
  const unsigned g = lsb_k_spmv_grid(LSB_SPMV_SELL, n, nitem, 0, grid_cap && grid_cap < res ? grid_cap : res);
  if (npartials)
    *npartials = g;
  if (period < NXCD || !plan || pold == pnew)
    errx(EXIT_FAILURE, "lsb_k_pcg_col_px: no column plan (period %u) or one direction buffer", period);
#define LSB_PX(NF)                                                                                    \
  do {                                                                                                \
    if (xupd)                                                                                         \
      k_pcg_col_px<NF, 3, true><<<g, WG, 0, s>>>(plan, period, n, sptr, mask, td, sbase, vals, vconst, r, pold, pnew, x, dc, \
                                                 partials, st, parity, parts2, nparts2);              \
    else                                                                                              \
      k_pcg_col_px<NF, 3, false><<<g, WG, 0, s>>>(plan, period, n, sptr, mask, td, sbase, vals, vconst, r, pold, pnew, x, \
                                                  dc, partials, st, parity, parts2, nparts2);         \
  } while (0)
  switch (nfar) {
  case 1: LSB_PX(1); break;
  case 2: LSB_PX(2); break;
  default: errx(EXIT_FAILURE, "lsb_k_pcg_col_px: %u far slots per side", nfar);
  }
#undef LSB_PX
}

void lsb_k_pcg_col_r(unsigned grid_cap, unsigned period, const unsigned *plan, unsigned nitem, unsigned n,
                     const unsigned *sptr, const unsigned long long *mask, const struct lsb_sell_tmpl *td, unsigned nfar,
                     const int *sbase, const double *vals, const double *vconst, const double *p, double *r, double dc,
                     struct lsb_pcg_state *st, int parity, int pbuf, int xtwo, const double *pq_parts, unsigned npq,
                     double *partials2, unsigned *npartials, void *stream) {
  hipStream_t s = (hipStream_t)stream;
  const unsigned g = lsb_k_spmv_grid(LSB_SPMV_SELL, n, nitem, 0, grid_cap && grid_cap < 1280u ? grid_cap : 1280u);
  *npartials = g;
  if (period < NXCD || !plan)
    errx(EXIT_FAILURE, "lsb_k_pcg_col_r: no column plan (period %u)", period);
  switch (nfar) {
  case 1:
    k_pcg_col_r<1><<<g, WG, 0, s>>>(plan, period, n, sptr, mask, td, sbase, vals, vconst, p, r, dc, st, parity, pbuf,
                                    xtwo, pq_parts, npq, partials2);
    break;
  case 2:
    k_pcg_col_r<2><<<g, WG, 0, s>>>(plan, period, n, sptr, mask, td, sbase, vals, vconst, p, r, dc, st, parity, pbuf,
                                    xtwo, pq_parts, npq, partials2);
    break;
  default: errx(EXIT_FAILURE, "lsb_k_pcg_col_r: %u far slots per side", nfar);
  }
}

void lsb_k_pcg_xfix(unsigned n, const double *p0, const double *p1, double *x, const struct lsb_pcg_state *st,
                    void *stream) {
  k_pcg_xfix<<<lsb_k_blas1_grid(n), WG, 0, (hipStream_t)stream>>>(n, p0, p1, x, st);
}

void lsb_k_cg1_update(unsigned n, double *u, const double *w, const double *dinv, double dc,
                      double *p,
                      double *s, double *x, double *r, struct lsb_pcg_state *st, int parity,
                      const double *parts_gr, unsigned ngr, const double *parts_d, unsigned nd,
                      const struct lsb_ar_collect *collect, double *partials2,
                      unsigned *npartials, void *stream) {
  const unsigned g = lsb_k_blas1_grid(n);
  *npartials = g;
  hipStream_t hs = (hipStream_t)stream;
  lsb_ar_collect col;
  memset(&col, 0, sizeof col);
  if (collect)
    col = *collect;
  const bool v2 = aligned16(u) && aligned16(w) && aligned16(dinv) && aligned16(p) &&
                  aligned16(s) && aligned16(x) && aligned16(r);
#define LSB_CG1(V, N, U)                                                                  \
  k_cg1_update<V, N, U><<<g, WG, 0, hs>>>(n, u, w, dinv, dc, p, s, x, r, st, parity, parts_gr, \
                                          ngr, parts_d, nd, col, partials2)
  if (!u) {
    if (dinv)
      errx(EXIT_FAILURE, "lsb_k_cg1_update: implicit u needs a constant diagonal");
    if (v2 && (g_blas1_nt & 32))
      LSB_CG1(true, true, true);
    else if (v2)
      LSB_CG1(true, false, true);
    else
      LSB_CG1(false, false, true);
  } else if (v2 && (g_blas1_nt & 32))
    LSB_CG1(true, true, false);
  else if (v2)
    LSB_CG1(true, false, false);
  else
    LSB_CG1(false, false, false);
#undef LSB_CG1
}

void lsb_k_pcg_update_p(unsigned n, const double *r, const double *dinv, double dc,
                        const double *pin, double *p, struct lsb_pcg_state *st, int parity,
                        const double *parts2, unsigned nparts2, void *stream) {
  const unsigned g = lsb_k_blas1_grid(n);
  const int x2 = 1;
  hipStream_t s = (hipStream_t)stream;
#define LSB_UPD_P(V2, NTR, NTP, X2) \
  k_pcg_update_p<V2, NTR, NTP, X2><<<g, WG, 0, s>>>(n, r, dinv, dc, pin, p, st, parity, parts2, nparts2)
#define LSB_UPD_P2(NTR, NTP)          \
  do {                                \
    if (big)                          \
      LSB_UPD_P(true, NTR, NTP, true); \
    else                              \
      LSB_UPD_P(true, NTR, NTP, false); \
  } while (0)
  if (aligned16(r) && aligned16(dinv) && aligned16(p) && aligned16(pin)) {
    const bool big = x2 && (size_t)n / 2 > (size_t)g * WG;
    switch ((g_blas1_nt >> 3) & 3) {
    case 0: LSB_UPD_P2(false, false); break;
    case 1: LSB_UPD_P2(true, false); break;
    case 2: LSB_UPD_P2(false, true); break;
    default: LSB_UPD_P2(true, true); break;
    }
  } else {
    LSB_UPD_P(false, false, false, false);
  }
#undef LSB_UPD_P2
#undef LSB_UPD_P
}

}
```

### lsbench_amd/csrc/hip_solver.c

```c
#define _GNU_SOURCE
#include "hip_solver.h"
#define NXCD_HOST 8u

unsigned pow2_ceil(unsigned v) {
  unsigned p = 1;
  while (p < v)
    p <<= 1;
  return p;
}

void choose_spmv(struct shard *s, const struct lsb_hip_opts *o) {
  const unsigned mean = s->n ? (unsigned)((s->nnz + s->n - 1) / s->n) : 1;
  int v = o->spmv_variant;
  if (v == LSB_SPMV_AUTO)
    v = s->nnz <= 500000ull ? LSB_SPMV_SUBWAVE : LSB_SPMV_ADAPTIVE;
  if (v == LSB_SPMV_PANEL && !s->pn)
    v = LSB_SPMV_ADAPTIVE;
  if (v == LSB_SPMV_BINNED && !s->bn)
    v = LSB_SPMV_ADAPTIVE;
  if (v == LSB_SPMV_TWOPHASE && !s->tp_bins)
    v = LSB_SPMV_ADAPTIVE;
  if (v == LSB_SPMV_SELL && !s->d_sptr)
    v = LSB_SPMV_ADAPTIVE;
  s->variant = v;
// ... 164 lines not shown
    unsigned char *ext = (unsigned char *)calloc(s->nblk ? s->nblk : 1, 1);
    for (unsigned k = 0; k < s->nblk; k++)
      for (unsigned r = rb[k]; r < rb[k + 1] && !ext[k]; r++)
        if (offs[r + 1] > offs[r] &&
            (cols[offs[r]] < (int)row_begin || cols[offs[r + 1] - 1] >= row_end))
          ext[k] = 1;
    while (b1 < s->nblk && ext[b1])
      b1++;
    while (b2 > b1 && ext[b2 - 1])
      b2--;
    for (unsigned k = b1; k < b2; k++)
      ok &= !ext[k];
    free(ext);
    s->ov_ok = ok && b2 > b1, s->ov_b1 = b1, s->ov_b2 = b2;
  }
  {
    struct csr gview = {n, 0, (unsigned *)offs, (unsigned *)cols, (double *)(S->vals + j0)};
    const char *e = getenv("LSBENCH_HIP_PANEL_COLS");
    const unsigned width = e ? (unsigned)strtoul(e, NULL, 10) : 524288u;
    const int forced = o->spmv_variant == LSB_SPMV_PANEL;
    const int scattered = s->nnz > 4000000ull && (double)(hi - lo) * 8.0 > 16.0e6 &&
                          lsb_csr_mean_scatter(&gview, row_begin) > 1.0e6;
    if (width && forced)
      shard_build_panels(s, &gview, width);
    if (width && (o->spmv_variant == LSB_SPMV_BINNED ||
                  (o->spmv_variant == LSB_SPMV_AUTO && scattered)))
      shard_build_bins(s, &gview, width);
    if (o->spmv_variant == LSB_SPMV_TWOPHASE ||
        (o->spmv_variant == LSB_SPMV_AUTO && scattered))
      shard_build_twophase(s, &gview, n_glob);
  }
  {
    struct csr gview = {n, 0, (unsigned *)offs, (unsigned *)cols, (double *)(S->vals + j0)};
    const int forced = o->spmv_variant == LSB_SPMV_SELL;
    const unsigned long long stored = (forced || s->nnz >= 4000000ull) ? lsb_csr_sell_stored(&gview) : 0;
    struct lsb_sell *E = NULL;
    if (stored && (forced || (o->spmv_variant == LSB_SPMV_AUTO && stored <= s->nnz + s->nnz / 8)))
      E = lsb_csr_sellize(&gview);
    if (E) {
      {
        unsigned bw = 0;
        for (unsigned i = 0; i < n; i++)
          if (offs[i + 1] > offs[i]) {
            const long long g = (long long)row_begin + i;
            const long long a = g - cols[offs[i]], b = (long long)cols[offs[i + 1] - 1] - g;
            if (a > (long long)bw)
              bw = (unsigned)a;
            if (b > (long long)bw)
              bw = (unsigned)b;
          }
        if (bw >= 64 * LSB_SELL_ROWS && bw % LSB_SELL_ROWS == 0 && E->nslice >= 2 * (bw / LSB_SELL_ROWS))
          s->sell_period = bw / LSB_SELL_ROWS;
        if (bw >= NXCD_HOST * LSB_SELL_ROWS && bw % LSB_SELL_ROWS == 0 && E->nslice >= 2 * (bw / LSB_SELL_ROWS))
          s->col_period = bw / LSB_SELL_ROWS;
      }
      s->nslice = E->nslice;
      s->sell32_bytes = (unsigned long long)E->stored * (s->mixed ? 8 : 12) + ((unsigned long long)E->nslice + 1) * 4;
      s->d_sptr = (unsigned *)dev_upload(E->sptr, ((size_t)E->nslice + 1) * sizeof(unsigned));
      s->d_scols = (int *)dev_upload(E->cols, ((size_t)E->stored + LSB_SELL_ROWS) * sizeof(int));
      s->d_svals = s->mixed ? (double *)upload_f32(E->vals, (size_t)E->stored + LSB_SELL_ROWS, NULL)
                            : (double *)dev_upload(E->vals, ((size_t)E->stored + LSB_SELL_ROWS) * sizeof(double));
      const int row_end = (int)(row_begin + n);
      unsigned s1 = 0, s2 = E->nslice;
      int ok = 1;
      unsigned char *ext = (unsigned char *)calloc(E->nslice ? E->nslice : 1, 1);
      for (unsigned k = 0; k < E->nslice; k++)
        for (unsigned r = k * LSB_SELL_ROWS; r < n && r < (k + 1) * LSB_SELL_ROWS && !ext[k]; r++)
          if (offs[r + 1] > offs[r] &&
              (cols[offs[r]] < (int)row_begin || cols[offs[r + 1] - 1] >= row_end))
            ext[k] = 1;
      while (s1 < E->nslice && ext[s1])
        s1++;
      while (s2 > s1 && ext[s2 - 1])
        s2--;
      for (unsigned k = s1; k < s2; k++)
        ok &= !ext[k];
      free(ext);
      s->ov_sok = ok && s2 > s1, s->ov_s1 = s1, s->ov_s2 = s2;
      LSB_CHK_HIP(hipStreamSynchronize(g_stream));
      lsb_sell_free(E);
      struct lsb_sell *H = getenv("LSBENCH_HIP_NO_C16") ? NULL : lsb_csr_sellize16(&gview, row_begin);
      if (H && H->stored > s->nnz + s->nnz / 8) {
        lsb_sell_free(H);
        H = NULL;
      }
      if (H) {
        s->d_sptr16 = (unsigned *)dev_upload(H->sptr, ((size_t)H->nslice + 1) * sizeof(unsigned));
        s->d_scodes = (short *)dev_upload(H->codes, ((size_t)H->ncode_slots + 1) * LSB_SELL_ROWS * sizeof(short));
        {
          unsigned ul = H->nslice ? (H->sptr[1] - H->sptr[0]) / LSB_SELL_ROWS : 0;
          for (unsigned k = 0; k < H->nslice && ul; k++)
            if ((H->sptr[k + 1] - H->sptr[k]) / LSB_SELL_ROWS != ul)
              ul = 0;
          s->sell_ulen = ul;
        }
        struct lsb_sell_vc *V = getenv("LSBENCH_HIP_NO_VCONST") ? NULL : lsb_sell16_value_slots(H);
        if (V && (unsigned long long)V->nval_slots * 8 > V->nslots * 7) {
          lsb_sell_vc_free(V);
          V = NULL;
        }
        if (V) {
          const size_t nv = ((size_t)V->nval_slots + 1) * LSB_SELL_ROWS;
          s->d_sbase = (int *)dev_upload(V->slots, 4 * ((size_t)V->nslots + 1) * sizeof(int));
          s->d_svconst = (double *)dev_upload(V->vconst, ((size_t)V->nslots + 1) * sizeof(double));
          s->d_svals16 = s->mixed ? (double *)upload_f32(V->vals, nv, NULL)
                                  : (double *)dev_upload(V->vals, nv * sizeof(double));
          s->sell_vslots = V->nval_slots, s->sell_slots = (unsigned)V->nslots;
          s->sell16_bytes = (unsigned long long)V->nslots * 24;
          struct lsb_sell_tmpls *TT = getenv("LSBENCH_HIP_NO_TMPL") ? NULL : lsb_sell16_templates(H, V);
          {
            char why[256];
            if (lsb_tmpl_check(H, V, TT, row_begin, n, n_glob, 0, why, sizeof why))
              errx(EXIT_FAILURE, "hip_cdna4: sliced-ELL layout breaks a bound its kernels rely on: %s", why);
          }
          if (TT) {
            if (s->mixed)
              for (unsigned t = 0; t < TT->ntmpl; t++)
                for (int j = 0; j < TT->t[t].nslots; j++)
                  TT->t[t].cst[j] = (double)(float)TT->t[t].cst[j];
            {
              unsigned *rec = lsb_calloc(unsigned, 4 * ((size_t)TT->nslice + 1));
              for (unsigned k = 0; k < TT->nslice; k++)
                rec[4 * (size_t)k] = TT->tid[k], rec[4 * (size_t)k + 1] = TT->vbase[2 * (size_t)k],
                               rec[4 * (size_t)k + 2] = TT->vbase[2 * (size_t)k + 1];
              s->d_srec = (unsigned *)dev_upload(rec, 4 * ((size_t)TT->nslice + 1) * sizeof(unsigned));
              LSB_CHK_HIP(hipStreamSynchronize(g_stream));
              free(rec);
            }
            s->d_tmask = (unsigned long long *)dev_upload(TT->mask, 2 * ((size_t)TT->nmask + 1) * sizeof(unsigned long long));
            s->d_tmpl = (struct lsb_sell_tmpl *)dev_upload(TT->t, (size_t)TT->ntmpl * sizeof(struct lsb_sell_tmpl));
            s->tmpl_nfar = TT->nfar, s->tmpl_count = TT->ntmpl;
            s->tmpl_pure = TT->covered, s->tmpl_shaped = TT->shaped;
            s->tmpl_bytes = 16ull * TT->nslice + (unsigned long long)TT->ntmpl * sizeof(struct lsb_sell_tmpl) +
                            16ull * TT->nmask +
                            TT->kept_read * LSB_SELL_ROWS * (s->mixed ? 4ull : 8ull);
            for (unsigned k = 0; k < H->nslice; k++)
              if (TT->tid[k] == 255)
                s->tmpl_bytes += (unsigned long long)(H->sptr[k + 1] - H->sptr[k]) / LSB_SELL_ROWS * 24 + 8;
            if (s->col_period && !getenv("LSBENCH_HIP_NO_COL")) {
              const char *ek = getenv("LSBENCH_HIP_COL_K");
              unsigned kauto = TT->nfar >= 2 ? TT->nslice / 5120u : TT->nslice / 15000u;
              kauto = kauto < 4u ? 4u : kauto > 16u ? 16u : kauto;
              const unsigned kmax = ek ? (unsigned)atoi(ek) : kauto;
              for (int w = 0; w < 2; w++) {
                if (w == 1 && !(s->d_colplan && s->ov_sok && (s->ov_s1 > 0 || s->ov_s2 < TT->nslice)))
                  break;
                struct lsb_tmpl_cols *CC = w == 0 ? lsb_sell_tmpl_columns(TT, s->col_period, kmax)
                                                  : lsb_sell_tmpl_columns_range(TT, s->col_period, kmax, s->ov_s1, s->ov_s2);
                if (!CC)
                  break;
                char why[256];
                if (lsb_tmpl_cols_check(TT, CC, why, sizeof why))
                  errx(EXIT_FAILURE, "hip_cdna4: z-column plan breaks a rule its kernel relies on: %s", why);
                unsigned *plan = lsb_calloc(unsigned, 16 + 4 * ((size_t)CC->nitem + 1));
                memcpy(plan, CC->xbeg, sizeof CC->xbeg);
                memcpy(plan + 16, CC->item, 4 * (size_t)CC->nitem * sizeof(unsigned));
                unsigned *d = (unsigned *)dev_upload(plan, (16 + 4 * ((size_t)CC->nitem + 1)) * sizeof(unsigned));
                LSB_CHK_HIP(hipStreamSynchronize(g_stream));
                free(plan);
                if (w == 0) {
                  s->d_colplan = d, s->col_items = CC->nitem, s->col_kmax = CC->kmax, s->col_centre0 = CC->centre0;
                  s->col_slices = CC->in_cols;
                  s->col_bytes = 16ull * CC->nitem + (unsigned long long)TT->ntmpl * sizeof(struct lsb_sell_tmpl);
                  for (unsigned q = 0; q < CC->nitem; q++) {
                    const unsigned sl = CC->item[4 * (size_t)q], run = CC->item[4 * (size_t)q + 1] & ~LSB_TMPL_COL_LOCKSTEP;
                    if (run >= 2) {
                      const struct lsb_sell_tmpl *t = &TT->t[TT->tid[sl]];
                      for (int j = 0; j < t->nslots; j++)
                        s->col_bytes += t->kind[j] == 2 ? 16ull : 0ull;
                    } else {
                      const unsigned q0 = H->sptr[sl] / LSB_SELL_ROWS, len = (H->sptr[sl + 1] - H->sptr[sl]) / LSB_SELL_ROWS;
                      s->col_bytes += 24ull * len + 8;
                      for (unsigned j = 0; j < len; j++)
                        if (V->slots[4 * ((size_t)q0 + j) + 2] >= 0)
                          s->col_bytes += LSB_SELL_ROWS * (s->mixed ? 4ull : 8ull);
                    }
                  }
                } else {
                  s->d_colplan_in = d, s->col_items_in = CC->nitem;
                  s->col_centre0 &= CC->centre0;
                }
                lsb_tmpl_cols_free(CC);
              }
            }
            LSB_CHK_HIP(hipStreamSynchronize(g_stream));
            lsb_sell_tmpls_free(TT);
          }
        } else {
          s->d_sbase = (int *)dev_upload(H->sbase, 2 * ((size_t)H->stored / LSB_SELL_ROWS + 1) * sizeof(int));
          s->d_svals16 = s->mixed ? (double *)upload_f32(H->vals, (size_t)H->stored + LSB_SELL_ROWS, NULL)
                                  : (double *)dev_upload(H->vals, ((size_t)H->stored + LSB_SELL_ROWS) * sizeof(double));
          s->sell_vslots = s->sell_slots = (unsigned)(H->stored / LSB_SELL_ROWS);
          s->sell16_bytes = (unsigned long long)s->sell_slots * 8;
        }
        s->sell16_bytes += (unsigned long long)H->ncode_slots * LSB_SELL_ROWS * sizeof(short) +
                           (unsigned long long)s->sell_vslots * LSB_SELL_ROWS * (s->mixed ? 4 : 8) +
                           (s->sell_ulen ? 0ull : ((unsigned long long)H->nslice + 1) * 4);

        LSB_CHK_HIP(hipStreamSynchronize(g_stream));
        lsb_sell_vc_free(V);
        lsb_sell_free(H);
      }
    }
  }
  precond_shard_blocks(s, offs, cols, S->vals + j0, o);
  LSB_CHK_HIP(hipStreamSynchronize(g_stream));
  free(rb), free(offs), free(cols), free(lanes);

  {
    size_t cnt = 3 * (size_t)n + n_glob;
    if (n_glob > n || o->nvirt > 1 || o->krylov == LSB_KRYLOV_PCG1)
      cnt += 2 * (size_t)n;
    if (o->precond == LSB_PRECOND_CHEBYSHEV)
      cnt += 2 * (size_t)n_glob + (size_t)n;
    else if (o->precond == LSB_PRECOND_BLOCKJACOBI)
      cnt += (size_t)n;
    else if (o->precond == LSB_PRECOND_FSAI)
      cnt += 4 * (size_t)n;
    if (o->krylov != LSB_KRYLOV_GMRES && !getenv("LSBENCH_HIP_NO_SLAB") && (size_t)n * sizeof(double) <= ((size_t)160 << 20)) {
      s->slab_cap = cnt * sizeof(double) + 16 * 256;
      if (hipMalloc((void **)&s->d_slab, s->slab_cap) != hipSuccess)
        s->d_slab = NULL, s->slab_cap = 0, (void)hipGetLastError();
    }
  }
  s->d_r = shard_vec(s, n);
  s->d_q = shard_vec(s, n);
  s->d_pfull = shard_vec(s, n_glob);
  s->d_dinv = shard_vec(s, n);
  LSB_CHK_HIP(hipMemsetAsync(s->d_pfull, 0, (size_t)n_glob * sizeof(double), g_stream));
  s->d_parts_pq = (double *)lsb_hip_malloc(3 * LSB_MAX_PARTIALS * sizeof(double));
  s->d_parts2 = (double *)lsb_hip_malloc(4 * LSB_MAX_PARTIALS * sizeof(double));
  s->d_st = (struct lsb_pcg_state *)lsb_hip_malloc(sizeof(struct lsb_pcg_state));
  LSB_CHK_HIP(hipMemsetAsync(s->d_st, 0, sizeof(struct lsb_pcg_state), g_stream));
  s->d_st_aux = (struct lsb_pcg_state *)lsb_hip_malloc(sizeof(struct lsb_pcg_state));
  LSB_CHK_HIP(hipMemsetAsync(s->d_st_aux, 0, sizeof(struct lsb_pcg_state), g_stream));
  choose_spmv(s, o);

  if (o->precond == LSB_PRECOND_JACOBI || o->precond == LSB_PRECOND_L1JACOBI ||
      o->precond == LSB_PRECOND_CHEBYSHEV) {
    int *d_nz = (int *)lsb_hip_malloc(sizeof(int)), nz = 0;
    LSB_CHK_HIP(hipMemsetAsync(d_nz, 0, sizeof(int), g_stream));
    if (o->precond == LSB_PRECOND_L1JACOBI)
      lsb_k_l1_setup(n, s->d_offs, s->d_vals, s->d_dinv, d_nz, g_stream);
    else
      lsb_k_jacobi_setup(n, row_begin, s->d_offs, s->d_cols, s->d_vals, s->d_dinv, d_nz,
                         g_stream);
    LSB_CHK_HIP(hipMemcpyAsync(&nz, d_nz, sizeof(int), hipMemcpyDeviceToHost, g_stream));
    LSB_CHK_HIP(hipStreamSynchronize(g_stream));
    lsb_hip_free(d_nz);
    if (nz)
      errx(EXIT_FAILURE, "hip_cdna4: %d rows have no non-zero %s; "
                         "Jacobi preconditioning needs one (cf. the stored-diagonal "
                         "assumption of src/cholmod-impl.h:13)", nz,
           o->precond == LSB_PRECOND_L1JACOBI ? "entry" : "diagonal entry");
  } else {
    double *ones = (double *)malloc((size_t)(n ? n : 1) * sizeof(double));
    for (unsigned i = 0; i < n; i++)
      ones[i] = 1.0;
    LSB_CHK_HIP(hipMemcpy(s->d_dinv, ones, (size_t)n * sizeof(double), hipMemcpyHostToDevice));
    free(ones);
  }
  if (n && !getenv("LSBENCH_HIP_NO_UNIFORM_DINV")) {
    double *h = (double *)malloc((size_t)n * sizeof(double));
    LSB_CHK_HIP(hipMemcpy(h, s->d_dinv, (size_t)n * sizeof(double), hipMemcpyDeviceToHost));
    int same = 1;
    for (unsigned i = 1; i < n && same; i++)
      same = h[i] == h[0];
    s->dinv_uniform = same, s->dinv_const = h[0];
    free(h);
  }
}

void shard_free(struct shard *s) {
  lsb_hip_free(s->d_offs), lsb_hip_free(s->d_cols), lsb_hip_free(s->d_vals), lsb_hip_free(s->d_vals32);
  lsb_hip_free(s->d_rowblk), lsb_hip_free(s->d_blklanes);
  shard_vec_free(s, s->d_dinv), shard_vec_free(s, s->d_r);
  shard_vec_free(s, s->d_q), shard_vec_free(s, s->d_pfull), lsb_hip_free(s->d_parts_pq);
  shard_vec_free(s, s->d_p1), shard_vec_free(s, s->d_s1);
  lsb_hip_free(s->d_parts2), lsb_hip_free(s->d_st), lsb_hip_free(s->d_st_aux);
  lsb_hip_free(s->pd_offs), lsb_hip_free(s->pd_cols), lsb_hip_free(s->pd_vals);
  lsb_hip_free(s->pd_rowmap), lsb_hip_free(s->pd_rowblk), lsb_hip_free(s->pd_blklanes);
  lsb_hip_free(s->d_sptr), lsb_hip_free(s->d_scols), lsb_hip_free(s->d_svals);
  lsb_hip_free(s->d_sptr16), lsb_hip_free(s->d_scodes), lsb_hip_free(s->d_sbase);
  lsb_hip_free(s->d_svals16), lsb_hip_free(s->d_svconst);
  lsb_hip_free(s->d_srec), lsb_hip_free(s->d_tmpl), lsb_hip_free(s->d_tmask), lsb_hip_free(s->d_colplan), lsb_hip_free(s->d_colplan_in);
  free(s->h_pblk);
  lsb_hip_free(s->bd_chunk), lsb_hip_free(s->bd_rows), lsb_hip_free(s->bd_cols);
  lsb_hip_free(s->bd_vals);
  free(s->h_binchunk);
  lsb_hip_free(s->tp_item), lsb_hip_free(s->tp_binptr), lsb_hip_free(s->tp_first);
  lsb_hip_free(s->tp_mask), lsb_hip_free(s->tp_delta);
  lsb_hip_free(s->tp_colw), lsb_hip_free(s->tp_roww), lsb_hip_free(s->tp_vals);
  lsb_hip_free(s->tp_prod), lsb_hip_free(s->tp_binparts);
  precond_free_shard(s);
  lsb_hip_free(s->d_slab);
  s->d_slab = NULL;
  free(s->recv), free(s->send);
}

void plan_exchange(struct shard *s, int me, int nall, const unsigned *hull) {
  s->recv = lsb_calloc(struct lsb_xfer, nall);
  s->send = lsb_calloc(struct lsb_xfer, nall);
  lsb_plan_exchange(me, nall, hull, s->recv, &s->nrecv, s->send, &s->nsend);
}

lsb_hip_solver *solver_alloc(int nshard, const struct lsb_hip_opts *o) {
  lsb_hip_solver *sv = lsb_calloc(lsb_hip_solver, 1);
  sv->nshard = nshard;
  sv->sh = lsb_calloc(struct shard, nshard);
  sv->o = *o;
// ... 320 lines not shown
  const unsigned f32 = s->mixed ? LSB_SP_F32 : 0u;
  const int col_all = s->d_colplan && s0 == 0 && ns == s->nslice;
  const int col_in = s->d_colplan_in && s0 == s->ov_s1 && ns == s->ov_s2 - s->ov_s1;
  if ((s->sp_flags & LSB_SP_C16) && (s->sp_flags & LSB_SP_TMPL) && (s->sp_flags & LSB_SP_COL) && (col_all || col_in) &&
      s->d_srec && s->d_scodes && !s->epi.zout)
    lsb_k_spmv_tmpl_col(s->sp_flags | f32, s->sp_grid, s->col_period, col_all ? s->d_colplan : s->d_colplan_in,
                        col_all ? s->col_items : s->col_items_in, s->col_centre0, s->n,
                        s->row_begin, s->n_glob, s->d_sptr16, s->d_tmask, s->d_tmpl, s->tmpl_nfar, s->d_sbase,
                        s->d_svals16, s->d_svconst, xfull, y, xdot, partials, np, st, &s->tail, g_stream);
  else if ((s->sp_flags & LSB_SP_C16) && (s->sp_flags & LSB_SP_TMPL) && s->d_srec && s->d_scodes)
    lsb_k_spmv_tmpl(s->sp_flags | f32, (s->sp_flags & LSB_SP_COL) ? 1536u : s->sp_grid, s->sp_period, s->d_sptr16, s0, ns, s->n, s->row_begin, s->n_glob,
                    s->d_srec, s->d_tmask, s->d_tmpl, s->tmpl_nfar, s->d_sbase, s->d_svals16, s->d_svconst, xfull, y, xdot, partials, np, st,
                    &s->tail, &s->epi, g_stream);
  else if ((s->sp_flags & LSB_SP_C16) && s->d_scodes)
    lsb_k_spmv_sell(s->sp_flags | f32, s->sp_grid, s->sp_period, s->d_sptr16, s0, ns, s->n, s->row_begin, s->n_glob, s->d_scodes,
                    s->d_sbase, s->d_svals16, s->d_svconst, s->sell_ulen, xfull, y, xdot, partials, np, st, &s->tail, &s->epi,
                    g_stream);
  else
    lsb_k_spmv_sell((s->sp_flags & ~LSB_SP_C16) | f32, s->sp_grid, s->sp_period, s->d_sptr, s0, ns, s->n, s->row_begin, s->n_glob,
                    s->d_scols, NULL, s->d_svals, NULL, 0, xfull, y, xdot, partials, np, st, &s->tail, NULL, g_stream);
}

void spmv_shard(struct shard *s, const double *xfull, double *y,
                       const double *xdot, double *partials, unsigned *np,
                       const struct lsb_pcg_state *st) {
  if (s->variant == LSB_SPMV_PANEL) {
    LSB_CHK_HIP(hipMemsetAsync(y, 0, (size_t)s->n * sizeof(double), g_stream));
    for (unsigned p = 0; p < s->pn; p++) {
      const unsigned b0 = s->h_pblk[p], nb = s->h_pblk[p + 1] - b0;
      if (nb)
        lsb_k_spmv(LSB_SPMV_ADAPTIVE, s->n, s->pd_offs, s->pd_cols, s->pd_vals,
                   s->pd_rowblk + b0, s->pd_blklanes + b0, nb, s->lanes, s->sp_flags,
                   s->sp_grid, xfull, y, NULL, NULL, NULL, st, s->pd_rowmap, NULL, g_stream);
    }
    if (partials)
      lsb_k_dot(s->n, y, xdot, partials, np, g_stream);
    return;
  }
  if (s->variant == LSB_SPMV_SELL) {
    sell_launch(s, 0, s->nslice, xfull, y, xdot, partials, np, st);
    return;
  }
  if (s->variant == LSB_SPMV_TWOPHASE) {
    lsb_k_spmv_twophase(s->tp_items, s->tp_item, s->tp_vals, s->tp_colw, s->tp_first, s->tp_mask,
                        s->tp_delta, s->tp_roww, s->tp_col_lo, s->tp_cols, s->tp_rows, s->tp_bins,
                        s->tp_binptr, s->tp_prod, s->n, xfull, s->tp_xlen, y, xdot, partials, np,
                        s->tp_binparts, st, g_stream);
    return;
  }
  if (s->variant == LSB_SPMV_BINNED) {
    LSB_CHK_HIP(hipMemsetAsync(y, 0, (size_t)s->n * sizeof(double), g_stream));
    for (unsigned b = 0; b < s->bn; b++)
      lsb_k_spmv_binned(s->sp_flags, s->bcap, s->bd_chunk, s->h_binchunk[b],
                        s->h_binchunk[b + 1] - s->h_binchunk[b], s->bd_rows, s->bd_cols, s->bd_vals,
                        xfull, y, st, g_stream);
    if (partials)
      lsb_k_dot(s->n, y, xdot, partials, np, g_stream);
    return;
  }
  const int f32 = s->mixed && (s->variant == LSB_SPMV_ADAPTIVE || s->variant == LSB_SPMV_SUBWAVE);
  lsb_k_spmv(s->variant, s->n, s->d_offs, s->d_cols, f32 ? (const double *)s->d_vals32 : s->d_vals,
             s->d_rowblk, s->d_blklanes, s->nblk, s->lanes, s->sp_flags | (f32 ? LSB_SP_F32 : 0u),
             s->sp_grid, xfull, y, xdot, partials, np, st, NULL, &s->tail, g_stream);
}

void spmv_shard_exact(struct shard *s, const double *xfull, double *y, const double *xdot,
                      double *partials, unsigned *np, const struct lsb_pcg_state *st) {
  if (!s->mixed) {
    spmv_shard(s, xfull, y, xdot, partials, np, st);
    return;
  }
  const int v = s->nnz <= 500000ull ? LSB_SPMV_SUBWAVE : LSB_SPMV_ADAPTIVE;
  lsb_k_spmv(v, s->n, s->d_offs, s->d_cols, s->d_vals, s->d_rowblk, s->d_blklanes, s->nblk, s->lanes,
             LSB_SP_PREFETCH | LSB_SP_NT, 0, xfull, y, xdot, partials, np, st, NULL, NULL, g_stream);
}

void tune_spmv(lsb_hip_solver *sv, struct shard *s) {
  const struct lsb_hip_opts *o = &sv->o;
  s->sp_flags = LSB_SP_PREFETCH | LSB_SP_NT;
  s->sp_grid = o->spmv_grid > 0 ? (unsigned)o->spmv_grid : LSB_MAX_PARTIALS;
  if (getenv("LSBENCH_HIP_FORCE_PERIOD"))
    s->sp_period = s->sell_period;
  if (o->spmv_tune >= 0) {
    s->sp_flags = (unsigned)o->spmv_tune & (31u | LSB_SP_TMPL | LSB_SP_DEFER | LSB_SP_COL);
    return;
  }
  if (s->variant == LSB_SPMV_SELL && !s->d_sptr)
    s->variant = LSB_SPMV_ADAPTIVE;
  if ((s->variant != LSB_SPMV_ADAPTIVE && s->variant != LSB_SPMV_PANEL &&
       s->variant != LSB_SPMV_SELL && s->variant != LSB_SPMV_BINNED &&
       s->variant != LSB_SPMV_TWOPHASE) ||
      s->nnz < 4000000ull)
    return;
  float best = 1e30f;
  unsigned bf = s->sp_flags, np;
  int bv = s->variant;
  const unsigned grid0 = s->sp_grid;
  unsigned bg = grid0, bp = 0;
  struct {
    int v;
    unsigned f, g, p;
  } cand[32];
  memset(cand, 0, sizeof cand);
  int ncand = 0;
  const int any = o->spmv_variant == LSB_SPMV_AUTO;
#define CAND(V, F, G, P)                                                                       \
  do {                                                                                         \
    if (ncand >= (int)(sizeof cand / sizeof cand[0]))                                          \
      errx(EXIT_FAILURE, "hip_cdna4: SpMV timing pass: candidate table too small");            \
    cand[ncand].v = (V), cand[ncand].f = (F), cand[ncand].g = (G), cand[ncand].p = (P), ncand++; \
  } while (0)
  if (any || s->variant == LSB_SPMV_ADAPTIVE)
    for (unsigned f = 0; f < 4; f++)
      CAND(LSB_SPMV_ADAPTIVE, f, grid0, 0);
  if (s->pn && (any || s->variant == LSB_SPMV_PANEL))
    for (unsigned f = 0; f < 4; f++)
      CAND(LSB_SPMV_PANEL, f, grid0, 0);
  if (s->tp_bins && (any || s->variant == LSB_SPMV_TWOPHASE))
    CAND(LSB_SPMV_TWOPHASE, 0, grid0, 0);
  if (s->bn && (any || s->variant == LSB_SPMV_BINNED)) {
    static const unsigned bf[] = {LSB_SP_NT, 0};
    for (unsigned k = 0; k < sizeof bf / sizeof bf[0]; k++)
      CAND(LSB_SPMV_BINNED, bf[k], grid0, 0);
  }
  const int periodic = s->sell_period != 0;
  if (s->d_sptr && (any || s->variant == LSB_SPMV_SELL))
    for (unsigned c16 = 0; c16 <= (s->d_scodes ? LSB_SP_C16 : 0u); c16 += LSB_SP_C16) {
      CAND(LSB_SPMV_SELL, c16 | LSB_SP_NT, grid0, 0);
      CAND(LSB_SPMV_SELL, c16, grid0, 0);
      if (o->spmv_grid <= 0)
        CAND(LSB_SPMV_SELL, c16 | LSB_SP_NT, 1536, 0);
      if (periodic) {
        CAND(LSB_SPMV_SELL, c16 | LSB_SP_NT, grid0, s->sell_period);
        CAND(LSB_SPMV_SELL, c16, grid0, s->sell_period);
      }
      if (c16 && s->d_srec) {
        const unsigned f = c16 | LSB_SP_NT | LSB_SP_TMPL;
        CAND(LSB_SPMV_SELL, f, grid0, 0);
        if (o->spmv_grid <= 0)
          CAND(LSB_SPMV_SELL, f, 1536, 0);
        if (periodic) {
          CAND(LSB_SPMV_SELL, f, grid0, s->sell_period);
          if (o->spmv_grid <= 0)
            CAND(LSB_SPMV_SELL, f, 1536, s->sell_period);
        }
        if (s->tmpl_nfar >= 1 && s->nnz >= 16000000ull) {
          const unsigned fd = f | LSB_SP_DEFER, gd = o->spmv_grid <= 0 ? 1536u : grid0;
          CAND(LSB_SPMV_SELL, fd, gd, 0);
          if (periodic)
            CAND(LSB_SPMV_SELL, fd, gd, s->sell_period);
        }
        if (s->d_colplan) {
          if (o->spmv_grid <= 0) {
            CAND(LSB_SPMV_SELL, f | LSB_SP_COL, 768, 0);
            CAND(LSB_SPMV_SELL, f | LSB_SP_COL, 1024, 0);
            CAND(LSB_SPMV_SELL, f | LSB_SP_COL, 1536, 0);
          } else
            CAND(LSB_SPMV_SELL, f | LSB_SP_COL, grid0, 0);
        }
      }
    }
#undef CAND
  for (int ci = 0; ci < ncand; ci++) {
    s->variant = cand[ci].v, s->sp_flags = cand[ci].f, s->sp_grid = cand[ci].g, s->sp_period = cand[ci].p;
    spmv_shard(s, s->d_pfull, s->d_q, s->d_pfull + s->row_begin, s->d_parts_pq, &np, NULL);
    LSB_CHK_HIP(hipEventRecord(sv->ev_t0, g_stream));
    const int reps = 5;
    for (int r = 0; r < reps; r++)
      spmv_shard(s, s->d_pfull, s->d_q, s->d_pfull + s->row_begin, s->d_parts_pq, &np, NULL);
    LSB_CHK_HIP(hipEventRecord(sv->ev_t1, g_stream));
    LSB_CHK_HIP(hipEventSynchronize(sv->ev_t1));
    float ms = 0.f;
    LSB_CHK_HIP(hipEventElapsedTime(&ms, sv->ev_t0, sv->ev_t1));
    ms *= 3.0f / reps;
    if (o->verbose > 1)
      fprintf(stderr, "hip_cdna4: spmv tune form=%d flags=%u grid=%u period=%u: %.1f us\n", s->variant,
              s->sp_flags, s->sp_grid, s->sp_period, ms * 1e3f / 3);
    if (!(s->sp_flags & LSB_SP_NT))
      ms *= 1.03f;
    if ((s->sp_flags & LSB_SP_COL) && s->d_colplan && sv->nshard == 1 && !sv->dist && !sv->multi && s->dinv_uniform &&
        !s->mixed && o->precond == LSB_PRECOND_JACOBI && (o->krylov == LSB_KRYLOV_PCG || o->krylov == LSB_KRYLOV_AUTO) &&
        !sv->env_no_fuse_px)
      ms *= 0.85f;
    if (ms < best)
      best = ms, bf = s->sp_flags, bv = s->variant, bg = s->sp_grid, bp = s->sp_period;
  }
  s->sp_grid = bg;
  s->sp_period = bp;
  s->variant = bv;
  s->sp_flags = bf;
  if (any && bv != LSB_SPMV_TWOPHASE && s->tp_bins) {
    lsb_hip_free(s->tp_item), lsb_hip_free(s->tp_binptr), lsb_hip_free(s->tp_first);
    lsb_hip_free(s->tp_mask), lsb_hip_free(s->tp_delta);
    lsb_hip_free(s->tp_colw), lsb_hip_free(s->tp_roww), lsb_hip_free(s->tp_vals);
    lsb_hip_free(s->tp_prod), lsb_hip_free(s->tp_binparts);
    s->tp_item = s->tp_binptr = s->tp_first = s->tp_delta = NULL, s->tp_mask = NULL;
    s->tp_colw = s->tp_roww = NULL;
    s->tp_vals = s->tp_prod = s->tp_binparts = NULL, s->tp_bins = 0;
  }
  if (any && bv != LSB_SPMV_BINNED && s->bn) {
    lsb_hip_free(s->bd_chunk), lsb_hip_free(s->bd_rows), lsb_hip_free(s->bd_cols);
    lsb_hip_free(s->bd_vals);
    s->bd_chunk = s->bd_rows = s->bd_cols = NULL, s->bd_vals = NULL, s->bn = 0;
  }
  if (!(bv == LSB_SPMV_SELL && (bf & LSB_SP_C16))) {
    lsb_hip_free(s->d_sptr16), lsb_hip_free(s->d_scodes), lsb_hip_free(s->d_sbase);
    lsb_hip_free(s->d_svals16), lsb_hip_free(s->d_svconst);
    s->d_sptr16 = NULL, s->d_scodes = NULL, s->d_sbase = NULL, s->d_svals16 = NULL, s->d_svconst = NULL;
  }
  if (!(bv == LSB_SPMV_SELL && (bf & LSB_SP_TMPL))) {
    lsb_hip_free(s->d_srec), lsb_hip_free(s->d_tmpl), lsb_hip_free(s->d_tmask);
    s->d_srec = NULL, s->d_tmpl = NULL, s->d_tmask = NULL;
  }
  if (!(bv == LSB_SPMV_SELL && (bf & LSB_SP_COL))) {
    lsb_hip_free(s->d_colplan), lsb_hip_free(s->d_colplan_in);
    s->d_colplan = s->d_colplan_in = NULL;
  }
  if (any && !(bv == LSB_SPMV_SELL && !(bf & LSB_SP_C16))) {
    lsb_hip_free(s->d_scols), lsb_hip_free(s->d_svals);
    s->d_scols = NULL, s->d_svals = NULL;
    if (bv != LSB_SPMV_SELL)
      lsb_hip_free(s->d_sptr), s->d_sptr = NULL;
  }
}

int lsb_hip_solver_spmv_dev(lsb_hip_solver *sv, const double *d_x, double *d_y) {
  if (!lsb_initialized)
    return 1;
  if (!sv || !d_x || !d_y)
    return 2;
  double *d_yout = NULL;
  if (sv->d_perm) {
    lsb_k_perm_gather(sv->n_here, sv->d_perm, d_x, sv->d_bp, g_stream);
    d_x = sv->d_bp, d_yout = d_y, d_y = sv->d_xp;
  }
  for (int i = 0; i < sv->nshard; i++) {
    struct shard *s = &sv->sh[i];
    LSB_CHK_HIP(hipMemcpyAsync(s->d_pfull + s->row_begin, d_x + (s->row_begin - sv->row_first),
                               (size_t)s->n * sizeof(double), hipMemcpyDeviceToDevice,
                               g_stream));
  }
  if (sv->multi)
    exchange_p(sv, 0);
  for (int i = 0; i < sv->nshard; i++) {
    struct shard *s = &sv->sh[i];
    spmv_shard_exact(s, s->d_pfull, d_y + (s->row_begin - sv->row_first), NULL, NULL, NULL, NULL);
  }
  if (d_yout)
    lsb_k_perm_scatter(sv->n_here, sv->d_perm, d_y, d_yout, g_stream);
  drain_stream(sv, "lsb_hip_solver_spmv_dev");
  check_aux_status(sv, "lsb_hip_solver_spmv_dev");
  return 0;
}

int lsb_hip_solver_time_spmv(lsb_hip_solver *sv, int warm, int reps, double *ms_avg) {
  if (!lsb_initialized)
    return 1;
  if (!sv || reps < 1 || !ms_avg)
    return 2;
  struct shard *s = &sv->sh[0];
  unsigned np;
  for (int i = 0; i < warm; i++)
    spmv_shard(s, s->d_pfull, s->d_q, s->d_pfull + s->row_begin, s->d_parts_pq, &np, NULL);
  LSB_CHK_HIP(hipEventRecord(sv->ev_t0, g_stream));
  for (int i = 0; i < reps; i++)
    spmv_shard(s, s->d_pfull, s->d_q, s->d_pfull + s->row_begin, s->d_parts_pq, &np, NULL);
  LSB_CHK_HIP(hipEventRecord(sv->ev_t1, g_stream));
  LSB_CHK_HIP(hipEventSynchronize(sv->ev_t1));
  float ms = 0.f;
  LSB_CHK_HIP(hipEventElapsedTime(&ms, sv->ev_t0, sv->ev_t1));
  *ms_avg = (double)ms / reps;
  return 0;
}

int lsb_hip_solver_jacobi_sweep_dev(lsb_hip_solver *sv, double w, const double *d_b,
                                    double *d_x) {
  if (!lsb_initialized)
    return 1;
  if (!sv || !d_b || !d_x)
    return 2;
  if (sv->d_perm) {
    lsb_k_perm_gather(sv->n_here, sv->d_perm, d_x, sv->d_xp, g_stream);
    lsb_k_perm_gather(sv->n_here, sv->d_perm, d_b, sv->d_bp, g_stream);
    for (int i = 0; i < sv->nshard; i++) {
      struct shard *s = &sv->sh[i];
      LSB_CHK_HIP(hipMemcpyAsync(s->d_pfull + s->row_begin, sv->d_xp + (s->row_begin - sv->row_first),
                                 (size_t)s->n * sizeof(double), hipMemcpyDeviceToDevice, g_stream));
    }
    if (sv->multi)
      exchange_p(sv, 0);
    for (int i = 0; i < sv->nshard; i++) {
      struct shard *s = &sv->sh[i];
      const size_t o = s->row_begin - sv->row_first;
      spmv_shard_exact(s, s->d_pfull, sv->d_tmp + o, NULL, NULL, NULL, NULL);
      lsb_k_jacobi_sweep(s->n, w, s->d_dinv, sv->d_bp + o, sv->d_tmp + o, sv->d_xp + o, g_stream);
    }
    lsb_k_perm_scatter(sv->n_here, sv->d_perm, sv->d_xp, d_x, g_stream);
    drain_stream(sv, "lsb_hip_solver_jacobi_sweep_dev");
    check_aux_status(sv, "lsb_hip_solver_jacobi_sweep_dev");
    return 0;
  }
  int rc = lsb_hip_solver_spmv_dev(sv, d_x, sv->d_tmp);
  if (rc)
    return rc;
  for (int i = 0; i < sv->nshard; i++) {
    struct shard *s = &sv->sh[i];
    const size_t o = s->row_begin - sv->row_first;
    lsb_k_jacobi_sweep(s->n, w, s->d_dinv, d_b + o, sv->d_tmp + o, d_x + o, g_stream);
  }
// ... 4 lines not shown
```

### lsbench_amd/csrc/lsb_operator.c

```c
#include "lsb_impl.h"
#include <string.h>
#ifdef _OPENMP
#include <omp.h>
#else
static inline int omp_get_max_threads(void) { return 1; }
#endif

static struct csr *csr_alloc(unsigned nrows, unsigned long long nnz) {
  if (nnz > 0xFFFFFFFFull)
    errx(EXIT_FAILURE, "CSR with %llu non-zeros does not fit 32-bit offsets "
                       "(reference layout, src/lsbench-impl.h:22-26)", nnz);
  struct csr *S = lsb_calloc(struct csr, 1);
  S->nrows = nrows, S->base = 0;
  S->offs = lsb_calloc(unsigned, (size_t)nrows + 1);
  S->cols = lsb_calloc(unsigned, (size_t)nnz);
  S->vals = lsb_calloc(double, (size_t)nnz);
  if (!S->offs || !S->cols || !S->vals)
    errx(EXIT_FAILURE, "out of host memory for a %u-row / %llu-nnz CSR", nrows, nnz);
  return S;
}

void lsb_csr_free(struct csr *A) {
  if (!A)
    return;
// ... 1194 lines not shown
  free(count);
  if (T->covered * 8 < (unsigned long long)ns * 7 || T->shaped * 4 < (unsigned long long)ns * 3) {
    lsb_sell_tmpls_free(T);
    return NULL;
  }
  return T;
}

int lsb_tmpl_check(const struct lsb_sell *S, const struct lsb_sell_vc *V, const struct lsb_sell_tmpls *T,
                   unsigned row_begin, unsigned nrows, unsigned xlen, int deep, char *why, size_t whylen) {
#define TC_FAIL(code, ...)                                                                     \
  do {                                                                                         \
    if (why && whylen)                                                                         \
      snprintf(why, whylen, __VA_ARGS__);                                                      \
    return code;                                                                               \
  } while (0)
  if (!S || !V || !S->sptr)
    TC_FAIL(1, "no layout");
  const unsigned ns = S->nslice;
  if ((unsigned long long)ns * LSB_SELL_ROWS < nrows || V->nslots != S->stored / LSB_SELL_ROWS)
    TC_FAIL(2, "%u slices for %u rows, %llu slot records for %llu slots", ns, nrows, V->nslots,
            S->stored / LSB_SELL_ROWS);
  if (T && T->nslice != ns)
    TC_FAIL(3, "templates of %u slices for a copy of %u", T->nslice, ns);
  if (T && (T->ntmpl > 254 || T->nfar > 2))
    TC_FAIL(4, "%u templates (at most 254), %u far slots per side (at most 2)", T->ntmpl, T->nfar);
  for (unsigned s = 0; s < ns; s++) {
    const unsigned q0 = S->sptr[s] / LSB_SELL_ROWS, len = (S->sptr[s + 1] - S->sptr[s]) / LSB_SELL_ROWS;
    const long long g0 = (long long)row_begin + (long long)s * LSB_SELL_ROWS;
    if (S->sptr[s + 1] < S->sptr[s] || S->sptr[s] % LSB_SELL_ROWS || (unsigned long long)q0 + len > V->nslots)
      TC_FAIL(5, "slice %u: slots [%u, %u + %u) of %llu", s, q0, q0, len, V->nslots);
    const unsigned live = nrows - s * LSB_SELL_ROWS < LSB_SELL_ROWS ? nrows - s * LSB_SELL_ROWS : LSB_SELL_ROWS;
    for (unsigned j = 0; j < len; j++) {
      const int *r = V->slots + 4 * ((size_t)q0 + j);
      if (r[2] < 0) {
        if (r[1] >= 0)
          TC_FAIL(6, "slice %u slot %u: constant but with code slot %d", s, j, r[1]);
        if (g0 + r[0] < 0 || g0 + r[0] + LSB_SELL_ROWS > (long long)xlen)
          TC_FAIL(7, "slice %u slot %u: constant slot gathers x[%lld, %lld) of %u", s, j, g0 + r[0],
                  g0 + r[0] + LSB_SELL_ROWS, xlen);
        if (live < LSB_SELL_ROWS)
          TC_FAIL(8, "slice %u slot %u: constant in a slice that holds only %u rows", s, j, live);
        if (V->vconst[(size_t)q0 + j] == 0.0)
          TC_FAIL(9, "slice %u slot %u: constant 0 (padding is never constant)", s, j);
      } else {
        if ((unsigned)r[2] >= V->nval_slots)
          TC_FAIL(10, "slice %u slot %u: value slot %d of %u", s, j, r[2], V->nval_slots);
        if (r[1] >= 0 && (unsigned)r[1] >= S->ncode_slots)
          TC_FAIL(11, "slice %u slot %u: code slot %d of %u", s, j, r[1], S->ncode_slots);
        if (deep && r[1] < 0) {
          const double *v = V->vals + (size_t)r[2] * LSB_SELL_ROWS;
          for (unsigned l = 0; l < LSB_SELL_ROWS; l++)
            if (v[l] != 0.0 && (l >= live || g0 + l + r[0] < 0 || g0 + l + r[0] >= (long long)xlen))
              TC_FAIL(12, "slice %u slot %u row %u: entry at column %lld of %u (rows in the slice: %u)", s, j, l,
                      g0 + l + r[0], xlen, live);
        }
      }
    }
    if (!T || T->tid[s] == 255)
      continue;
    if (T->tid[s] >= T->ntmpl)
      TC_FAIL(13, "slice %u: template %u of %u", s, T->tid[s], T->ntmpl);
    const struct lsb_sell_tmpl *t = &T->t[T->tid[s]];
    if (t->nslots < 1 || t->nslots > LSB_TMPL_SLOTS || (unsigned)t->nslots != len)
      TC_FAIL(14, "slice %u: template of %d slots for a slice of %u", s, t->nslots, len);
    const int nf = (int)T->nfar, c = nf + 1;
    if (t->shaped && (t->nslots != 2 * nf + 3 || t->base[c - 1] != t->base[c] - 1 || t->base[c + 1] != t->base[c] + 1))
      TC_FAIL(15, "slice %u: shaped template without the [%d][c-1, c, c+1][%d] shape", s, nf, nf);
    const unsigned vb = T->vbase[2 * (size_t)s], mb = T->vbase[2 * (size_t)s + 1];
    for (int j = 0; j < t->nslots; j++) {
      const int *r = V->slots + 4 * ((size_t)q0 + j);
      if (j && t->base[j] <= t->base[j - 1])
        TC_FAIL(16, "slice %u: template bases not ascending at slot %d", s, j);
      if (t->base[j] != r[0] || r[1] >= 0)
        TC_FAIL(17, "slice %u slot %d: template base %d, slot record {%d, %d}", s, j, t->base[j], r[0], r[1]);
      const int side = t->shaped && (j == c - 1 || j == c + 1);
      if (t->kind[j] != 0 && !side)
        TC_FAIL(18, "slice %u slot %d: kind %d outside the slots c-1 / c+1 of a shaped template", s, j, t->kind[j]);
      if (t->kind[j] == 0) {
        if (t->kidx[j] != -1 || r[2] >= 0 || memcmp(&t->cst[j], &V->vconst[(size_t)q0 + j], sizeof(double)))
          TC_FAIL(19, "slice %u slot %d: template constant %g, slot record {value slot %d, constant %g}", s, j,
                  t->cst[j], r[2], V->vconst[(size_t)q0 + j]);
      } else if (t->kind[j] == 1) {
        if (t->kidx[j] < 0 || (unsigned long long)vb + (unsigned)t->kidx[j] >= V->nval_slots ||
            r[2] != (int)(vb + (unsigned)t->kidx[j]))
          TC_FAIL(20, "slice %u slot %d: kept slot %u + %d, slot record names %d of %u", s, j, vb, t->kidx[j], r[2],
                  V->nval_slots);
      } else if (t->kind[j] == 2) {
        if (t->kidx[j] < 0 || (unsigned long long)mb + (unsigned)t->kidx[j] >= T->nmask || r[2] < 0 ||
            (unsigned)r[2] >= V->nval_slots || t->cst[j] == 0.0)
          TC_FAIL(21, "slice %u slot %d: mask %u + %d of %llu (value slot %d, number %g)", s, j, mb, t->kidx[j],
                  T->nmask, r[2], t->cst[j]);
        if (deep) {
          const unsigned long long *m = T->mask + 2 * ((size_t)mb + (unsigned)t->kidx[j]);
          const double *v = V->vals + (size_t)r[2] * LSB_SELL_ROWS;
          for (unsigned l = 0; l < LSB_SELL_ROWS; l++) {
            const double want = (m[l >> 6] >> (l & 63u)) & 1ull ? t->cst[j] : 0.0;
            if (memcmp(&want, &v[l], sizeof want) && !(want == 0.0 && v[l] == 0.0))
              TC_FAIL(22, "slice %u slot %d row %u: mask gives %g, the slot holds %g", s, j, l, want, v[l]);
          }
        }
      } else
        TC_FAIL(23, "slice %u slot %d: kind %d", s, j, t->kind[j]);
    }
  }
  return 0;
#undef TC_FAIL
}

#define LSB_COL_XCDS 8

static int col_member(const struct lsb_sell_tmpls *T, unsigned s, unsigned period) {
  if (T->tid[s] == 255 || T->nfar < 1)
    return 0;
  const struct lsb_sell_tmpl *t = &T->t[T->tid[s]];
  const int c = (int)T->nfar + 1, last = 2 * (int)T->nfar + 2;
  if (!t->shaped || t->nslots != last + 1)
    return 0;
  for (int j = 0; j < t->nslots; j++)
    if (t->kind[j] == 1)
      return 0;
  const long long plane = (long long)LSB_SELL_ROWS * period;
  return (long long)t->base[0] == (long long)t->base[c] - plane && (long long)t->base[last] == (long long)t->base[c] + plane;
}
static int col_same(const struct lsb_sell_tmpls *T, unsigned a, unsigned b) {
  if (T->tid[a] != T->tid[b])
    return 0;
  const struct lsb_sell_tmpl *t = &T->t[T->tid[a]];
  size_t nmk = 0;
  for (int j = 0; j < t->nslots; j++)
    nmk += t->kind[j] == 2;
  return !nmk || !memcmp(T->mask + 2 * (size_t)T->vbase[2 * (size_t)a + 1], T->mask + 2 * (size_t)T->vbase[2 * (size_t)b + 1],
                         2 * nmk * sizeof(unsigned long long));
}

struct lsb_tmpl_cols *lsb_sell_tmpl_columns(const struct lsb_sell_tmpls *T, unsigned period, unsigned kmax) {
  return lsb_sell_tmpl_columns_range(T, period, kmax, 0, T ? T->nslice : 0);
}

struct lsb_tmpl_cols *lsb_sell_tmpl_columns_range(const struct lsb_sell_tmpls *T, unsigned period, unsigned kmax,
                                                  unsigned s_lo, unsigned s_hi) {
  if (!T || period < LSB_COL_XCDS || T->nslice < 2 * period || T->nfar < 1 || s_hi > T->nslice || s_lo >= s_hi)
    return NULL;
  if (kmax < 2)
    kmax = 2;
  if (kmax > LSB_TMPL_COL_MAX)
    kmax = LSB_TMPL_COL_MAX;
  const unsigned ns = T->nslice, nplanes = (ns + period - 1) / period;
  struct lsb_tmpl_cols *C = lsb_calloc(struct lsb_tmpl_cols, 1);
  C->kmax = kmax, C->period = period, C->centre0 = 1, C->s_lo = s_lo, C->s_hi = s_hi;
  C->item = lsb_calloc(unsigned, 4 * ((size_t)ns + 1));
  const unsigned ngroups = (nplanes + kmax - 1) / kmax;
  const unsigned long long ncell = (unsigned long long)ngroups * period, total = s_hi - s_lo;
  unsigned ni = 0, xk = 0;
  unsigned long long seen = 0;
  C->xbeg[0] = 0;
  for (unsigned long long cell = 0; cell < ncell; cell++) {
    const unsigned zg = (unsigned)(cell / period), p = (unsigned)(cell % period);
    const unsigned z0 = (unsigned)((unsigned long long)nplanes * zg / ngroups),
                   zend = (unsigned)((unsigned long long)nplanes * (zg + 1) / ngroups);
    while (xk + 1 < LSB_COL_XCDS && seen * LSB_COL_XCDS >= total * (xk + 1))
      C->xbeg[++xk] = ni;
    for (unsigned z = z0; z < zend;) {
      const unsigned long long s = (unsigned long long)z * period + p;
      if (s >= s_hi)
        break;
      if (s < s_lo) {
        z++;
        continue;
      }
      unsigned run = 1;
      if (col_member(T, (unsigned)s, period))
        while (z + run < zend && s + (unsigned long long)run * period < s_hi &&
               col_member(T, (unsigned)(s + (unsigned long long)run * period), period) &&
               col_same(T, (unsigned)s, (unsigned)(s + (unsigned long long)run * period)))
          run++;
      unsigned *it = C->item + 4 * (size_t)ni++;
      it[0] = (unsigned)s, it[1] = run, it[2] = T->tid[s], it[3] = T->vbase[2 * (size_t)s + 1];
      if (run >= 2) {
        C->in_cols += run;
        C->centre0 &= T->t[T->tid[s]].base[T->nfar + 1] == 0;
      }
      seen += run;
      z += run;
    }
  }
  while (xk + 1 < LSB_COL_XCDS)
    C->xbeg[++xk] = ni;
  C->xbeg[LSB_COL_XCDS] = C->nitem = ni;
  for (unsigned k = 0; k < LSB_COL_XCDS; k++)
    for (unsigned i = C->xbeg[k]; i + 4 <= C->xbeg[k + 1]; i += 4) {
      const unsigned *it = C->item + 4 * (size_t)i;
      if (it[1] >= 2 && it[5] == it[1] && it[9] == it[1] && it[13] == it[1])
        for (int w = 0; w < 4; w++)
          C->item[4 * (size_t)(i + w) + 1] |= LSB_TMPL_COL_LOCKSTEP;
    }
  if (C->in_cols * 4 < (unsigned long long)(s_hi - s_lo) * 3) {
    lsb_tmpl_cols_free(C);
    return NULL;
  }
  return C;
}

int lsb_tmpl_cols_check(const struct lsb_sell_tmpls *T, const struct lsb_tmpl_cols *C, char *why, size_t whylen) {
#define CC_FAIL(code, ...)                                                                     \
  do {                                                                                         \
    if (why && whylen)                                                                         \
      snprintf(why, whylen, __VA_ARGS__);                                                      \
    free(seen);                                                                                \
    return code;                                                                               \
  } while (0)
  unsigned char *seen = NULL;
  if (!T || !C || !C->item)
    CC_FAIL(1, "no column plan");
  const unsigned ns = T->nslice, period = C->period;
  if (C->s_hi > ns || C->s_lo >= C->s_hi)
    CC_FAIL(11, "slices [%u, %u) of %u", C->s_lo, C->s_hi, ns);
  if (period < LSB_COL_XCDS || C->kmax < 2 || C->kmax > LSB_TMPL_COL_MAX || C->xbeg[0] != 0 || C->xbeg[LSB_COL_XCDS] != C->nitem)
    CC_FAIL(2, "period %u, columns of up to %u slices, items [%u, %u) of %u", period, C->kmax, C->xbeg[0],
            C->xbeg[LSB_COL_XCDS], C->nitem);
  for (unsigned k = 0; k < LSB_COL_XCDS; k++)
    if (C->xbeg[k] > C->xbeg[k + 1])
      CC_FAIL(3, "item ranges of the XCDs not ascending at %u", k);
  seen = (unsigned char *)calloc((size_t)ns + 1, 1);
  if (!seen)
    CC_FAIL(4, "out of memory");
  for (unsigned i = 0; i < C->nitem; i++) {
    const unsigned *it = C->item + 4 * (size_t)i;
    const unsigned s = it[0], run = it[1] & ~LSB_TMPL_COL_LOCKSTEP;
    if (it[1] & LSB_TMPL_COL_LOCKSTEP) {
      unsigned xk = 0;
      while (xk + 1 < LSB_COL_XCDS && C->xbeg[xk + 1] <= i)
        xk++;
      const unsigned g0 = C->xbeg[xk] + (i - C->xbeg[xk]) / 4 * 4;
      if (g0 + 4 > C->xbeg[xk + 1])
        CC_FAIL(12, "item %u: lockstep in a turn of fewer than four items", i);
      for (unsigned w = 0; w < 4; w++)
        if (C->item[4 * (size_t)(g0 + w) + 1] != it[1] || run < 2)
          CC_FAIL(12, "item %u: lockstep, but item %u of its turn has another length", i, g0 + w);
    }
    if (run < 1 || run > C->kmax || s < C->s_lo || (unsigned long long)s + (unsigned long long)(run - 1) * period >= C->s_hi)
      CC_FAIL(5, "item %u: %u slices from slice %u, every %u, of [%u, %u)", i, run, s, period, C->s_lo, C->s_hi);
    for (unsigned k = 0; k < run; k++) {
      const unsigned sk = s + k * period;
      if (seen[sk]++)
        CC_FAIL(6, "item %u: slice %u is in two items", i, sk);
      if (run >= 2 && (!col_member(T, sk, period) || !col_same(T, s, sk)))
        CC_FAIL(7, "item %u: slice %u does not continue the column of slice %u", i, sk, s);
    }
    if (run >= 2 && C->centre0 && T->t[T->tid[s]].base[T->nfar + 1] != 0)
      CC_FAIL(10, "item %u: centre base %d in a plan that says 0", i, T->t[T->tid[s]].base[T->nfar + 1]);
    if (run >= 2 && (it[2] != T->tid[s] || it[3] != T->vbase[2 * (size_t)s + 1]))
      CC_FAIL(8, "item %u: template %u / first mask %u, its first slice has %u / %u", i, it[2], it[3], T->tid[s],
              T->vbase[2 * (size_t)s + 1]);
  }
  for (unsigned s = C->s_lo; s < C->s_hi; s++)
    if (!seen[s])
      CC_FAIL(9, "slice %u is in no item", s);
  free(seen);
  return 0;
#undef CC_FAIL
}

void lsb_tmpl_cols_free(struct lsb_tmpl_cols *C) {
  if (!C)
    return;
  free(C->item), free(C);
}

void lsb_sell_tmpls_free(struct lsb_sell_tmpls *T) {
  if (!T)
    return;
  free(T->tid), free(T->vbase), free(T->mask), free(T->t), free(T);
}

void lsb_sell_vc_free(struct lsb_sell_vc *V) {
  if (!V)
    return;
  free(V->slots), free(V->vconst), free(V->vals), free(V);
}

void lsb_sell_free(struct lsb_sell *S) {
  if (!S)
    return;
  free(S->sptr), free(S->cols), free(S->vals), free(S->codes), free(S->sbase), free(S);
}
```

Baseline: 1.032.

## Walk odd z-group columns downward to reuse boundary planes across adjacent groups

```diff
diff --git a/include/lsbench_hip.h b/include/lsbench_hip.h
--- a/include/lsbench_hip.h
+++ b/include/lsbench_hip.h
@@ -225,6 +225,9 @@
 int lsb_tmpl_check(const struct lsb_sell *S, const struct lsb_sell_vc *V, const struct lsb_sell_tmpls *T,
                    unsigned row_begin, unsigned nrows, unsigned xlen, int deep, char *why, size_t whylen);
 #define LSB_TMPL_COL_MAX 16
+#define LSB_TMPL_COL_GRID(nfar) ((nfar) >= 2 ? 768u : 1280u)
+#define LSB_TMPL_COL_TURN(nfar) (4u * LSB_TMPL_COL_GRID(nfar) / 8u)
+#define LSB_TMPL_COL_DOWN 9
 #define LSB_TMPL_COL_LOCKSTEP 0x80000000u
 struct lsb_tmpl_cols {
   unsigned nitem, kmax, period;
@@ -233,6 +236,7 @@
   unsigned *item;
   unsigned long long in_cols;
   int centre0;
+  unsigned *down;
 };
 struct lsb_tmpl_cols *lsb_sell_tmpl_columns(const struct lsb_sell_tmpls *T, unsigned period, unsigned kmax);
 struct lsb_tmpl_cols *lsb_sell_tmpl_columns_range(const struct lsb_sell_tmpls *T, unsigned period, unsigned kmax,
diff --git a/lsbench_amd/_lib.py b/lsbench_amd/_lib.py
--- a/lsbench_amd/_lib.py
+++ b/lsbench_amd/_lib.py
@@ -99,7 +99,8 @@
 class TmplCols(C.Structure):
     _fields_ = [("nitem", C.c_uint), ("kmax", C.c_uint), ("period", C.c_uint), ("s_lo", C.c_uint), ("s_hi", C.c_uint),
                 ("xbeg", C.c_uint * 9),
-                ("item", C.POINTER(C.c_uint)), ("in_cols", C.c_ulonglong), ("centre0", C.c_int)]
+                ("item", C.POINTER(C.c_uint)), ("in_cols", C.c_ulonglong), ("centre0", C.c_int),
+                ("down", C.POINTER(C.c_uint))]
 
 
 class Binned(C.Structure):
diff --git a/lsbench_amd/csrc/hip_kernels.hip b/lsbench_amd/csrc/hip_kernels.hip
--- a/lsbench_amd/csrc/hip_kernels.hip
+++ b/lsbench_amd/csrc/hip_kernels.hip
@@ -1345,10 +1345,10 @@
 };
 template <int NF, int DOT>
 __device__ __forceinline__ void col_issue(col_ops<NF> &o, sell_d2u &cnext, const col_tmpl<NF> &T, const double *__restrict__ x,
-                                          const double *__restrict__ xdot, long long gu, unsigned lrow, unsigned P,
+                                          const double *__restrict__ xdot, long long gu, unsigned lrow, long long D,
                                           unsigned xlen, unsigned lane, bool with_next) {
   if (with_next)
-    cnext = *(const sell_d2u *)(x + (gu + T.bc + (long long)P) + 2 * lane);
+    cnext = *(const sell_d2u *)(x + (gu + T.bc + D) + 2 * lane);
 #pragma unroll
   for (int k = 0; k < NF - 1; k++) {
     o.lo[k] = *(const sell_d2u *)(x + (gu + T.bl[k]) + 2 * lane);
@@ -1387,6 +1387,9 @@
 }
 
 #define LSB_COL_HEAD 16
+__device__ __forceinline__ bool col_walks_down(const unsigned *__restrict__ plan, unsigned dofs, unsigned it) {
+  return dofs && ((plan[dofs + (it >> 5)] >> (it & 31u)) & 1u);
+}
 template <int NF, int DOT>
 __global__ __launch_bounds__(WG, DOT == 2 ? 5 : 6) void k_spmv_tmpl_col(
     const unsigned *__restrict__ plan, unsigned period, unsigned n, unsigned row_begin, unsigned xlen,
@@ -1401,6 +1404,7 @@
   const unsigned gx = gridDim.x / NXCD, xcd = blockIdx.x % NXCD, slot = blockIdx.x / NXCD;
   const unsigned i0 = plan[xcd], i1 = plan[xcd + 1];
   const u4v *__restrict__ items = (const u4v *)(plan + LSB_COL_HEAD);
+  const unsigned dofs = plan[LSB_TMPL_COL_DOWN];
   const int stopped = st ? st->status : 0;
   const unsigned P = period * LSB_SELL_ROWS;
   double dot = 0.0;
@@ -1424,13 +1428,6 @@
         C.kl[k] = T->cst[1 + k], C.kh[k] = T->cst[NF + 3 + k];
       }
       const int side_k[2] = {T->kidx[NF], T->kidx[NF + 2]}, side_kd[2] = {T->kind[NF], T->kind[NF + 2]};
-      long long gu = (long long)s * LSB_SELL_ROWS + row_begin;
-      unsigned lrow = s * LSB_SELL_ROWS;
-      col_ops<NF> cur, nxt;
-      sell_d2u cm = *(const sell_d2u *)(x + (gu + C.bc - (long long)P) + 2 * lane);
-      sell_d2u c0 = *(const sell_d2u *)(x + (gu + C.bc) + 2 * lane);
-      sell_d2u cp, cn;
-      col_issue<NF, DOT>(cur, cp, C, x, xdot, gu, lrow, P, xlen, lane, true);
       unsigned long long mk[2][2] = {{0ull, 0ull}, {0ull, 0ull}};
 #pragma unroll
       for (int side = 0; side < 2; side++)
@@ -1438,37 +1435,50 @@
           const unsigned long long *mp = mask + 2 * ((size_t)mb + (unsigned)side_k[side]);
           mk[side][0] = mp[0], mk[side][1] = mp[1];
         }
+      const bool down = col_walks_down(plan, dofs, it);
+      const unsigned s0 = down ? s + (K - 1) * period : s;
+      const long long D = down ? -(long long)P : (long long)P;
+      const unsigned Du = (unsigned)D;
+      long long gu = (long long)s0 * LSB_SELL_ROWS + row_begin;
+      unsigned lrow = s0 * LSB_SELL_ROWS;
+      col_ops<NF> cur, nxt;
+      sell_d2u cb = *(const sell_d2u *)(x + (gu + C.bc - D) + 2 * lane);
+      sell_d2u c0 = *(const sell_d2u *)(x + (gu + C.bc) + 2 * lane);
+      sell_d2u ca, cn;
+      col_issue<NF, DOT>(cur, ca, C, x, xdot, gu, lrow, D, xlen, lane, true);
       double vm0 = T->cst[NF], vm1 = vm0, vp0 = T->cst[NF + 2], vp1 = vp0;
       if (side_k[0] >= 0 || side_k[1] >= 0)
         tmpl_side_values(T, NF, 0u, lane, side_k, side_kd, mk, vals, f32, vm0, vm1, vp0, vp1);
       if (stopped)
         return;
-      col_issue<NF, DOT>(nxt, cn, C, x, xdot, gu + (long long)P, lrow + P, P, xlen, lane, true);
+      col_issue<NF, DOT>(nxt, cn, C, x, xdot, gu + D, lrow + Du, D, xlen, lane, true);
       double a0, a1;
-      col_compute<NF, DOT>(cur, cm, c0, cp, C, vm0, vm1, vp0, vp1, lane, a0, a1, dot);
-      cm = c0, c0 = cp, cp = cn, cur = nxt;
+      col_compute<NF, DOT>(cur, down ? ca : cb, c0, down ? cb : ca, C, vm0, vm1, vp0, vp1, lane, a0, a1, dot);
+      cb = c0, c0 = ca, ca = cn, cur = nxt;
       for (unsigned k = 1; k + 1 < K; k++) {
-        gu += (long long)P, lrow += P;
+        gu += D, lrow += Du;
         if (lockstep)
           __builtin_amdgcn_s_barrier();
-        col_issue<NF, DOT>(nxt, cn, C, x, xdot, gu + (long long)P, lrow + P, P, xlen, lane, true);
+        col_issue<NF, DOT>(nxt, cn, C, x, xdot, gu + D, lrow + Du, D, xlen, lane, true);
         {
           const sell_d2v o = {a0, a1};
-          *(sell_d2v *)(y + (lrow - P) + 2 * lane) = o;
+          *(sell_d2v *)(y + (lrow - Du) + 2 * lane) = o;
         }
-        col_compute<NF, DOT>(cur, cm, c0, cp, C, vm0, vm1, vp0, vp1, lane, a0, a1, dot);
-        cm = c0, c0 = cp, cp = cn, cur = nxt;
-      }
-      gu += (long long)P, lrow += P;
+        col_compute<NF, DOT>(cur, down ? ca : cb, c0, down ? cb : ca, C, vm0, vm1, vp0, vp1, lane, a0, a1, dot);
+        cb = c0, c0 = ca, ca = cn, cur = nxt;
+      }
+      gu += D, lrow += Du;
       {
         const sell_d2v o = {a0, a1};
-        *(sell_d2v *)(y + (lrow - P) + 2 * lane) = o;
-      }
-      col_compute<NF, DOT>(cur, cm, c0, cp, C, vm0, vm1, vp0, vp1, lane, a0, a1, dot);
+        *(sell_d2v *)(y + (lrow - Du) + 2 * lane) = o;
+      }
+      col_compute<NF, DOT>(cur, down ? ca : cb, c0, down ? cb : ca, C, vm0, vm1, vp0, vp1, lane, a0, a1, dot);
       {
         const sell_d2v o = {a0, a1};
         *(sell_d2v *)(y + lrow + 2 * lane) = o;
       }
+      if (stopped)
+        return;
     } else {
       const unsigned row = s * LSB_SELL_ROWS + 2 * lane;
       const int grow = (int)(row + row_begin);
@@ -1534,18 +1544,18 @@
 template <int NF, bool WITH_X, int NT>
 __device__ __forceinline__ void colp_issue_c(colp_c<NF> &o, const col_tmpl<NF> &T, const double *__restrict__ r,
                                              const double *__restrict__ pold, const double *__restrict__ x,
-                                             const double *pstale, long long gu, unsigned P, unsigned xlen,
+                                             const double *pstale, long long gu, long long D, unsigned xlen,
                                              unsigned lane) {
-  const long long ga = gu + T.bc + (long long)P;
+  const long long ga = gu + T.bc + D;
   o.rn = *(const sell_d2u *)(r + ga + 2 * lane);
   o.pn = *(const sell_d2u *)(pold + ga + 2 * lane);
   if (WITH_X) {
     if (NT & 1) {
-      o.xn = __builtin_nontemporal_load((const sell_d2v *)(x + (gu + (long long)P) + 2 * lane));
-      o.sn = __builtin_nontemporal_load((const sell_d2v *)(pstale + (gu + (long long)P) + 2 * lane));
+      o.xn = __builtin_nontemporal_load((const sell_d2v *)(x + (gu + D) + 2 * lane));
+      o.sn = __builtin_nontemporal_load((const sell_d2v *)(pstale + (gu + D) + 2 * lane));
     } else {
-      o.xn = *(const sell_d2v *)(x + (gu + (long long)P) + 2 * lane);
-      o.sn = *(const sell_d2v *)(pstale + (gu + (long long)P) + 2 * lane);
+      o.xn = *(const sell_d2v *)(x + (gu + D) + 2 * lane);
+      o.sn = *(const sell_d2v *)(pstale + (gu + D) + 2 * lane);
     }
   }
   long long el = gu + T.bc - 1, er = gu + T.bc + (long long)LSB_SELL_ROWS;
@@ -1565,8 +1575,8 @@
   }
 }
 template <int NF, bool OWNED, bool XUPD>
-__device__ __forceinline__ void colp_compute(const colp_c<NF> &o, const colp_m<NF> &m, const sell_d2u &pm,
-                                             const sell_d2u &p0, sell_d2u &pp, const col_tmpl<NF> &T, double vm0,
+__device__ __forceinline__ void colp_compute(const colp_c<NF> &o, const colp_m<NF> &m, const sell_d2u &pb,
+                                             const sell_d2u &p0, sell_d2u &pp, bool down, const col_tmpl<NF> &T, double vm0,
                                              double vm1, double vp0, double vp1, double beta, double alpha, double alpha2,
                                              double dc, unsigned lane, colp_out &out, double &dot) {
   pp.x = pnew_of(dc, o.rn.x, beta, o.pn.x), pp.y = pnew_of(dc, o.rn.y, beta, o.pn.y);
@@ -1582,6 +1592,7 @@
     up = edge;
   if (lane == 63)
     dn = edge;
+  const sell_d2u &pm = down ? pp : pb, &pu = down ? pb : pp;
   double a0 = fma(T.k0, pm.x, 0.0), a1 = fma(T.k0, pm.y, 0.0);
 #pragma unroll
   for (int k = 0; k < NF - 1; k++) {
@@ -1596,7 +1607,7 @@
     const double h0 = pnew_of(dc, m.rhi[k].x, beta, m.phi[k].x), h1 = pnew_of(dc, m.rhi[k].y, beta, m.phi[k].y);
     a0 = fma(T.kh[k], h0, a0), a1 = fma(T.kh[k], h1, a1);
   }
-  a0 = fma(T.kL, pp.x, a0), a1 = fma(T.kL, pp.y, a1);
+  a0 = fma(T.kL, pu.x, a0), a1 = fma(T.kL, pu.y, a1);
   out.q.x = a0, out.q.y = a1;
   dot = fma(a0, p0.x, dot), dot = fma(a1, p0.y, dot);
 }
@@ -1660,13 +1671,13 @@
       COLP_ST(q + (LROW) + 2 * lane, (OUT).q, 2);                                              \
     if (WITH_XP) {                                                                             \
       if (XUPD)                                                                                \
-        COLP_ST(x + ((LROW) + P) + 2 * lane, (OUT).x, 1);                                      \
-      COLP_ST(pnew + ((LROW) + P) + 2 * lane, (OUT).p, 2);                                     \
+        COLP_ST(x + ((LROW) + Du) + 2 * lane, (OUT).x, 1);                                     \
+      COLP_ST(pnew + ((LROW) + Du) + 2 * lane, (OUT).p, 2);                                    \
     }                                                                                          \
   } while (0)
 
 template <int NF, int NT, bool XUPD>
-__global__ __launch_bounds__(WG, NF == 2 ? 3 : 4) void k_pcg_col_px(
+__global__ __launch_bounds__(WG, NF == 2 ? 3 : 5) void k_pcg_col_px(
     const unsigned *__restrict__ plan, unsigned period, unsigned n, const unsigned *__restrict__ sptr,
     const unsigned long long *__restrict__ mask, const lsb_sell_tmpl *__restrict__ td, const int *__restrict__ sbase,
     const double *__restrict__ vals, const double *__restrict__ vconst, const double *__restrict__ r,
@@ -1705,6 +1716,7 @@
     return;
   const double beta = rz_new / rz_old;
   const u4v *__restrict__ items = (const u4v *)(plan + LSB_COL_HEAD);
+  const unsigned dofs = plan[LSB_TMPL_COL_DOWN];
   const unsigned P = period * LSB_SELL_ROWS;
   double dot = 0.0;
   for (unsigned g = slot; i0 + 4 * g < i1; g += gx) {
@@ -1726,20 +1738,24 @@
         C.kl[k] = T->cst[1 + k], C.kh[k] = T->cst[NF + 3 + k];
       }
       const int side_k[2] = {T->kidx[NF], T->kidx[NF + 2]}, side_kd[2] = {T->kind[NF], T->kind[NF + 2]};
-      long long gu = (long long)s * LSB_SELL_ROWS;
-      unsigned lrow = s * LSB_SELL_ROWS;
+      const bool down = col_walks_down(plan, dofs, it);
+      const unsigned s0 = down ? s + (K - 1) * period : s;
+      const long long D = down ? -(long long)P : (long long)P;
+      const unsigned Du = (unsigned)D;
+      long long gu = (long long)s0 * LSB_SELL_ROWS;
+      unsigned lrow = s0 * LSB_SELL_ROWS;
       const long long gc = gu + C.bc;
-      const sell_d2u rb = *(const sell_d2u *)(r + (gc - (long long)P) + 2 * lane);
-      const sell_d2u pb = *(const sell_d2u *)(pold + (gc - (long long)P) + 2 * lane);
+      const sell_d2u rb = *(const sell_d2u *)(r + (gc - D) + 2 * lane);
+      const sell_d2u pb = *(const sell_d2u *)(pold + (gc - D) + 2 * lane);
       const sell_d2u r0 = *(const sell_d2u *)(r + gc + 2 * lane), o0 = *(const sell_d2u *)(pold + gc + 2 * lane);
-      sell_d2v x0 = {0.0, 0.0}, s0 = {0.0, 0.0};
+      sell_d2v x0 = {0.0, 0.0}, s0v = {0.0, 0.0};
       if (XUPD)
-        x0 = *(const sell_d2v *)(x + lrow + 2 * lane), s0 = *(const sell_d2v *)(pnew + lrow + 2 * lane);
+        x0 = *(const sell_d2v *)(x + lrow + 2 * lane), s0v = *(const sell_d2v *)(pnew + lrow + 2 * lane);
       colp_c<NF> c0, c1;
       colp_m<NF> m0, m1, m2;
-      colp_issue_c<NF, XUPD, NT>(c0, C, r, pold, x, pnew, gu, P, n, lane);
+      colp_issue_c<NF, XUPD, NT>(c0, C, r, pold, x, pnew, gu, D, n, lane);
       colp_issue_m<NF>(m0, C, r, pold, gu, lane);
-      colp_issue_m<NF>(m1, C, r, pold, gu + (long long)P, lane);
+      colp_issue_m<NF>(m1, C, r, pold, gu + D, lane);
       unsigned long long mk[2][2] = {{0ull, 0ull}, {0ull, 0ull}};
 #pragma unroll
       for (int side = 0; side < 2; side++)
@@ -1754,24 +1770,24 @@
       pm.x = pnew_of(dc, rb.x, beta, pb.x), pm.y = pnew_of(dc, rb.y, beta, pb.y);
       p0.x = pnew_of(dc, r0.x, beta, o0.x), p0.y = pnew_of(dc, r0.y, beta, o0.y);
       colp_out res;
-      res.x.x = (x0.x + alpha2 * s0.x) + alpha * o0.x, res.x.y = (x0.y + alpha2 * s0.y) + alpha * o0.y;
+      res.x.x = (x0.x + alpha2 * s0v.x) + alpha * o0.x, res.x.y = (x0.y + alpha2 * s0v.y) + alpha * o0.y;
       res.p.x = p0.x, res.p.y = p0.y;
       res.q = res.p;
-      COLP_STORE(res, lrow - P, false, true);
+      COLP_STORE(res, lrow - Du, false, true);
       for (unsigned k = 0; k + 2 < K; k++) {
-        colp_issue_c<NF, XUPD, NT>(c1, C, r, pold, x, pnew, gu + (long long)P, P, n, lane);
-        colp_issue_m<NF>(m2, C, r, pold, gu + 2 * (long long)P, lane);
-        colp_compute<NF, true, XUPD>(c0, m0, pm, p0, pp, C, vm0, vm1, vp0, vp1, beta, alpha, alpha2, dc, lane, res, dot);
+        colp_issue_c<NF, XUPD, NT>(c1, C, r, pold, x, pnew, gu + D, D, n, lane);
+        colp_issue_m<NF>(m2, C, r, pold, gu + 2 * D, lane);
+        colp_compute<NF, true, XUPD>(c0, m0, pm, p0, pp, down, C, vm0, vm1, vp0, vp1, beta, alpha, alpha2, dc, lane, res, dot);
         COLP_STORE(res, lrow, false, true);
         pm = p0, p0 = pp, c0 = c1, m0 = m1, m1 = m2;
-        gu += (long long)P, lrow += P;
-      }
-      colp_issue_c<NF, false, NT>(c1, C, r, pold, x, pnew, gu + (long long)P, P, n, lane);
-      colp_compute<NF, true, XUPD>(c0, m0, pm, p0, pp, C, vm0, vm1, vp0, vp1, beta, alpha, alpha2, dc, lane, res, dot);
+        gu += D, lrow += Du;
+      }
+      colp_issue_c<NF, false, NT>(c1, C, r, pold, x, pnew, gu + D, D, n, lane);
+      colp_compute<NF, true, XUPD>(c0, m0, pm, p0, pp, down, C, vm0, vm1, vp0, vp1, beta, alpha, alpha2, dc, lane, res, dot);
       COLP_STORE(res, lrow, false, true);
       pm = p0, p0 = pp, c0 = c1, m0 = m1;
-      gu += (long long)P, lrow += P;
-      colp_compute<NF, false, XUPD>(c0, m0, pm, p0, pp, C, vm0, vm1, vp0, vp1, beta, alpha, alpha2, dc, lane, res, dot);
+      gu += D, lrow += Du;
+      colp_compute<NF, false, XUPD>(c0, m0, pm, p0, pp, down, C, vm0, vm1, vp0, vp1, beta, alpha, alpha2, dc, lane, res, dot);
       COLP_STORE(res, lrow, false, false);
     } else {
       for (unsigned k = 0; k < K; k++)
@@ -1823,6 +1839,7 @@
     st->pq = pq, st->alpha[1] = st->alpha[0], st->alpha[0] = alpha, st->xpend = (xtwo ? 3 : 1) + pbuf;
   }
   const u4v *__restrict__ items = (const u4v *)(plan + LSB_COL_HEAD);
+  const unsigned dofs = plan[LSB_TMPL_COL_DOWN];
   const unsigned P = period * LSB_SELL_ROWS;
   double acc[2] = {0.0, 0.0}, nodot = 0.0;
 #define COLR_FINISH(A0, A1, RV, LROW)                                                          \
@@ -1854,13 +1871,17 @@
         C.kl[k] = T->cst[1 + k], C.kh[k] = T->cst[NF + 3 + k];
       }
       const int side_k[2] = {T->kidx[NF], T->kidx[NF + 2]}, side_kd[2] = {T->kind[NF], T->kind[NF + 2]};
-      long long gu = (long long)s * LSB_SELL_ROWS;
-      unsigned lrow = s * LSB_SELL_ROWS;
+      const bool down = col_walks_down(plan, dofs, it);
+      const unsigned s0 = down ? s + (K - 1) * period : s;
+      const long long D = down ? -(long long)P : (long long)P;
+      const unsigned Du = (unsigned)D;
+      long long gu = (long long)s0 * LSB_SELL_ROWS;
+      unsigned lrow = s0 * LSB_SELL_ROWS;
       col_ops<NF> cur, nxt;
-      sell_d2u cm = *(const sell_d2u *)(p + (gu + C.bc - (long long)P) + 2 * lane);
+      sell_d2u cb = *(const sell_d2u *)(p + (gu + C.bc - D) + 2 * lane);
       sell_d2u c0 = *(const sell_d2u *)(p + (gu + C.bc) + 2 * lane);
-      sell_d2u cp, cn;
-      col_issue<NF, 2>(cur, cp, C, p, r, gu, lrow, P, n, lane, true);
+      sell_d2u ca, cn;
+      col_issue<NF, 2>(cur, ca, C, p, r, gu, lrow, D, n, lane, true);
       unsigned long long mk[2][2] = {{0ull, 0ull}, {0ull, 0ull}};
 #pragma unroll
       for (int side = 0; side < 2; side++)
@@ -1872,15 +1893,15 @@
       if (side_k[0] >= 0 || side_k[1] >= 0)
         tmpl_side_values(T, NF, 0u, lane, side_k, side_kd, mk, vals, 0, vm0, vm1, vp0, vp1);
       for (unsigned k = 0; k + 1 < K; k++) {
-        col_issue<NF, 2>(nxt, cn, C, p, r, gu + (long long)P, lrow + P, P, n, lane, true);
+        col_issue<NF, 2>(nxt, cn, C, p, r, gu + D, lrow + Du, D, n, lane, true);
         double a0, a1;
-        col_compute<NF, 0>(cur, cm, c0, cp, C, vm0, vm1, vp0, vp1, lane, a0, a1, nodot);
+        col_compute<NF, 0>(cur, down ? ca : cb, c0, down ? cb : ca, C, vm0, vm1, vp0, vp1, lane, a0, a1, nodot);
         COLR_FINISH(a0, a1, cur.xd, lrow);
-        cm = c0, c0 = cp, cp = cn, cur = nxt;
-        gu += (long long)P, lrow += P;
+        cb = c0, c0 = ca, ca = cn, cur = nxt;
+        gu += D, lrow += Du;
       }
       double a0, a1;
-      col_compute<NF, 0>(cur, cm, c0, cp, C, vm0, vm1, vp0, vp1, lane, a0, a1, nodot);
+      col_compute<NF, 0>(cur, down ? ca : cb, c0, down ? cb : ca, C, vm0, vm1, vp0, vp1, lane, a0, a1, nodot);
       COLR_FINISH(a0, a1, cur.xd, lrow);
     } else {
       for (unsigned k = 0; k < K; k++) {
@@ -2540,7 +2561,7 @@
                       unsigned *npartials, struct lsb_pcg_state *st, int parity, const double *parts2,
                       unsigned nparts2, void *stream) {
   hipStream_t s = (hipStream_t)stream;
-  const unsigned res = nfar == 2 ? 768u : 1280u;
+  const unsigned res = LSB_TMPL_COL_GRID(nfar);
   const unsigned g = lsb_k_spmv_grid(LSB_SPMV_SELL, n, nitem, 0, grid_cap && grid_cap < res ? grid_cap : res);
   if (npartials)
     *npartials = g;
diff --git a/lsbench_amd/csrc/hip_solver.c b/lsbench_amd/csrc/hip_solver.c
--- a/lsbench_amd/csrc/hip_solver.c
+++ b/lsbench_amd/csrc/hip_solver.c
@@ -340,10 +340,15 @@
                 char why[256];
                 if (lsb_tmpl_cols_check(TT, CC, why, sizeof why))
                   errx(EXIT_FAILURE, "hip_cdna4: z-column plan breaks a rule its kernel relies on: %s", why);
-                unsigned *plan = lsb_calloc(unsigned, 16 + 4 * ((size_t)CC->nitem + 1));
+                const size_t nw = 16 + 4 * ((size_t)CC->nitem + 1), nd = CC->down ? ((size_t)CC->nitem + 31) / 32 : 0;
+                unsigned *plan = lsb_calloc(unsigned, nw + nd);
                 memcpy(plan, CC->xbeg, sizeof CC->xbeg);
                 memcpy(plan + 16, CC->item, 4 * (size_t)CC->nitem * sizeof(unsigned));
-                unsigned *d = (unsigned *)dev_upload(plan, (16 + 4 * ((size_t)CC->nitem + 1)) * sizeof(unsigned));
+                if (nd) {
+                  plan[LSB_TMPL_COL_DOWN] = (unsigned)nw;
+                  memcpy(plan + nw, CC->down, nd * sizeof(unsigned));
+                }
+                unsigned *d = (unsigned *)dev_upload(plan, (nw + nd) * sizeof(unsigned));
                 LSB_CHK_HIP(hipStreamSynchronize(g_stream));
                 free(plan);
                 if (w == 0) {
@@ -970,9 +975,12 @@
         }
         if (s->d_colplan) {
           if (o->spmv_grid <= 0) {
+            const unsigned gcol = LSB_TMPL_COL_GRID(s->tmpl_nfar);
             CAND(LSB_SPMV_SELL, f | LSB_SP_COL, 768, 0);
-            CAND(LSB_SPMV_SELL, f | LSB_SP_COL, 1024, 0);
-            CAND(LSB_SPMV_SELL, f | LSB_SP_COL, 1536, 0);
+            if (gcol > 768) {
+              CAND(LSB_SPMV_SELL, f | LSB_SP_COL, 1024, 0);
+              CAND(LSB_SPMV_SELL, f | LSB_SP_COL, gcol, 0);
+            }
           } else
             CAND(LSB_SPMV_SELL, f | LSB_SP_COL, grid0, 0);
         }
diff --git a/lsbench_amd/csrc/lsb_operator.c b/lsbench_amd/csrc/lsb_operator.c
--- a/lsbench_amd/csrc/lsb_operator.c
+++ b/lsbench_amd/csrc/lsb_operator.c
@@ -1370,6 +1370,8 @@
   C->item = lsb_calloc(unsigned, 4 * ((size_t)ns + 1));
   const unsigned ngroups = (nplanes + kmax - 1) / kmax;
   const unsigned long long ncell = (unsigned long long)ngroups * period, total = s_hi - s_lo;
+  if (2ull * period <= LSB_TMPL_COL_TURN(T->nfar))
+    C->down = lsb_calloc(unsigned, ((size_t)ns + 1 + 31) / 32);
   unsigned ni = 0, xk = 0;
   unsigned long long seen = 0;
   C->xbeg[0] = 0;
@@ -1393,6 +1395,8 @@
                col_member(T, (unsigned)(s + (unsigned long long)run * period), period) &&
                col_same(T, (unsigned)s, (unsigned)(s + (unsigned long long)run * period)))
           run++;
+      if (C->down && (zg & 1u) && run >= 3)
+        C->down[ni / 32] |= 1u << (ni % 32);
       unsigned *it = C->item + 4 * (size_t)ni++;
       it[0] = (unsigned)s, it[1] = run, it[2] = T->tid[s], it[3] = T->vbase[2 * (size_t)s + 1];
       if (run >= 2) {
@@ -1440,9 +1444,12 @@
   for (unsigned k = 0; k < LSB_COL_XCDS; k++)
     if (C->xbeg[k] > C->xbeg[k + 1])
       CC_FAIL(3, "item ranges of the XCDs not ascending at %u", k);
+  if (C->down && 2ull * period > LSB_TMPL_COL_TURN(T->nfar))
+    CC_FAIL(13, "walk directions on z-groups of %u cells, %u items per XCD and turn", period, LSB_TMPL_COL_TURN(T->nfar));
   seen = (unsigned char *)calloc((size_t)ns + 1, 1);
   if (!seen)
     CC_FAIL(4, "out of memory");
+  const unsigned nplanes = (ns + period - 1) / period, ngroups = (nplanes + C->kmax - 1) / C->kmax;
   for (unsigned i = 0; i < C->nitem; i++) {
     const unsigned *it = C->item + 4 * (size_t)i;
     const unsigned s = it[0], run = it[1] & ~LSB_TMPL_COL_LOCKSTEP;
@@ -1471,6 +1478,11 @@
     if (run >= 2 && (it[2] != T->tid[s] || it[3] != T->vbase[2 * (size_t)s + 1]))
       CC_FAIL(8, "item %u: template %u / first mask %u, its first slice has %u / %u", i, it[2], it[3], T->tid[s],
               T->vbase[2 * (size_t)s + 1]);
+    if (C->down) {
+      const unsigned zg = (unsigned)(((unsigned long long)(s / period + 1) * ngroups - 1) / nplanes);
+      if (((C->down[i / 32] >> (i % 32)) & 1u) != ((zg & 1u) && run >= 3))
+        CC_FAIL(13, "item %u: %u slices walk %s in z-group %u", i, run, ((zg & 1u) && run >= 3) ? "upward" : "downward", zg);
+    }
   }
   for (unsigned s = C->s_lo; s < C->s_hi; s++)
     if (!seen[s])
@@ -1483,7 +1495,7 @@
 void lsb_tmpl_cols_free(struct lsb_tmpl_cols *C) {
   if (!C)
     return;
-  free(C->item), free(C);
+  free(C->item), free(C->down), free(C);
 }
 
 void lsb_sell_tmpls_free(struct lsb_sell_tmpls *T) {
```

New measurement: 1.090 (median of 6 runs). 1.06x the previous value.
